# BloodAxe/segmentation-networks-benchmark

Measured on AMD Instinct MI355X. Metric: images/sec/GPU (fwd+bwd) ZF_UNET 224x224 bs=32; 1/2/4/8-GPU scaling, higher is better.
Workload: dtype bf16; 1 GPU; ZF_UNET 224x224 bf16 bs=32/GPU, bce_dice, SGD lr 1e-3, Dropout2d 0.2, train step torch_train.py:180-190 (configs[1]); global_batch=32, parallelism=dp1

## Files before the change

__graft_entry__.py:

```python
import os
import subprocess
import sys

ROOT = os.path.dirname(os.path.abspath(__file__))
PKG = os.path.join(ROOT, 'segmentation-networks-benchmark_amd')


def _paths():
    for p in (PKG, ROOT):
        if p not in sys.path:
            sys.path.insert(0, p)


def build():
    subprocess.check_call(['bash', os.path.join(PKG, 'csrc', 'build.sh')])
    _paths()
    import torch
    from segnb import _native as nv
    import ctypes
    lib = ctypes.CDLL(nv.LIB_PATH)
    for name in (list(nv.SIGNATURES) + list(nv.PLAIN) + list(nv.MC_SIGNATURES) + list(nv.MC_PLAIN) + list(nv.GCN_SIGNATURES)
                 + list(nv.GCN_PLAIN)):
        getattr(lib, name)
    import lib.models.zf_unet
    import lib.models.gcn
    import lib.losses
    import lib.metrics


def smoke():
    _paths()
    import torch
    from oracle import train_step_ref, zf_unet_ref
    from lib.models.zf_unet import ZF_UNET
    from lib.losses import BCEWithLogitsLossAndSmoothJaccard
    from segnb import _native as nv
    nv.load()
    dev = torch.device('cuda:0')
    B, S, F = 2, 64, 8
    x, y = train_step_ref.synthetic_batch(B, S, seed=21)
    sd = zf_unet_ref.default_init_state(filters=F, seed=5)
    ref_loss, ref_logits, ref_grads = train_step_ref.loss_and_grads(sd, x, y, 'bce_jaccard')
    torch.manual_seed(5)
    m = ZF_UNET(dropout_val=0.0, filters=F)
    m.set_compute_dtype('f32')
    m = m.to(dev).train()
    opt = torch.optim.SGD(m.parameters(), lr=1e-3)
    opt.zero_grad()
    out = m(x.to(dev))
    loss = BCEWithLogitsLossAndSmoothJaccard()(out, y.to(dev))
    (B * loss).backward()
    opt.step()
    torch.cuda.synchronize()
    dl = abs(loss.item() - ref_loss.item())
    assert dl < 1e-5, 'loss differs from the oracle by %g' % dl
    worst = 0.0
    for n, p in m.named_parameters():
        if n.endswith('.conv.bias'):
            assert float(p.grad.abs().max()) == 0.0
            continue
        r = ref_grads[n]
        worst = max(worst, float((p.grad.cpu() - r).abs().max() / (r.abs().max() + 1e-6)))
    assert worst < 2e-3, 'gradient differs from the oracle (rel %g)' % worst
    m2 = ZF_UNET(dropout_val=0.2, filters=F).to(dev).train()
    l2 = BCEWithLogitsLossAndSmoothJaccard()(m2(x.to(dev)), y.to(dev))
    (B * l2).backward()
    torch.cuda.synchronize()
    assert torch.isfinite(l2).item()
    print('smoke ok: |dloss| = %.2e, worst rel grad err = %.2e, bf16 loss = %.4f' % (dl, worst, l2.item()))


if __name__ == '__main__':
    build()
    if len(sys.argv) > 1 and sys.argv[1] == 'smoke':
        smoke()
```

segmentation-networks-benchmark_amd/csrc/common.h:

```cpp
#pragma once
#include <hip/hip_runtime.h>
#include <hip/hip_ext.h>
#include <stdint.h>
#include <stdio.h>
#include <string.h>

#include "../../include/segnb_hip.h"

typedef __attribute__((ext_vector_type(8))) __bf16 bf16x8_t;
typedef __attribute__((ext_vector_type(16))) float f32x16_t;

struct bf16_t {
    unsigned short bits;
};

void segnb_set_error(const char* fmt, ...);

#define SEGNB_CHECK_ARG(cond, msg)                                   \
    do {                                                             \
        if (!(cond)) {                                               \
            segnb_set_error("%s: bad argument: %s", __func__, msg);  \
            return SEGNB_E_BADARG;                                   \
        }                                                            \
    } while (0)
// ... 26 lines not shown
struct SegnbPlanScope {
    bool top;
    SegnbPlanScope();
    ~SegnbPlanScope();
};
template <class T>
inline T segnb_plan_keep(T v) {
    static_assert(!(std::is_pointer<T>::value && std::is_class<typename std::remove_pointer<T>::type>::value),
                  "segnb_plan_keep: add an overload that copies this struct into the plan");
    return v;
}
inline const segnb_conv_geom* segnb_plan_keep(const segnb_conv_geom* g) {
    return g ? (const segnb_conv_geom*)segnb_plan_dup(g, sizeof(*g)) : g;
}
inline const segnb_loss_spec* segnb_plan_keep(const segnb_loss_spec* g) {
    return g ? (const segnb_loss_spec*)segnb_plan_dup(g, sizeof(*g)) : g;
}
inline const segnb_bn_reduce_epilogue* segnb_plan_keep(const segnb_bn_reduce_epilogue* g) {
    return g ? (const segnb_bn_reduce_epilogue*)segnb_plan_dup(g, sizeof(*g)) : g;
}
inline const segnb_bn_apply_epilogue* segnb_plan_keep(const segnb_bn_apply_epilogue* g) {
    return g ? (const segnb_bn_apply_epilogue*)segnb_plan_dup(g, sizeof(*g)) : g;
}
inline const segnb_upcat_src* segnb_plan_keep(const segnb_upcat_src* g) {
    return g ? (const segnb_upcat_src*)segnb_plan_dup(g, sizeof(*g)) : g;
}
inline const segnb_operand_tf* segnb_plan_keep(const segnb_operand_tf* g) {
    return g ? (const segnb_operand_tf*)segnb_plan_dup(g, sizeof(*g)) : g;
}
inline const segnb_wgrad_target* segnb_plan_keep(const segnb_wgrad_target* g) {
    return g ? (const segnb_wgrad_target*)segnb_plan_dup(g, sizeof(*g)) : g;
}
inline const segnb_act_epilogue* segnb_plan_keep(const segnb_act_epilogue* g) {
    return g ? (const segnb_act_epilogue*)segnb_plan_dup(g, sizeof(*g)) : g;
}
template <class... P, class... A>
inline void segnb_plan_record_call(const char* name, int (*fn)(P...), A... args) {
    static_assert(sizeof...(P) == sizeof...(A), "argument count");
    std::tuple<P...> kept(segnb_plan_keep((P)args)...);
    segnb_plan_push([fn, kept]() { return std::apply(fn, kept); }, name);
}
extern int g_segnb_census_on;
void segnb_census(const char* name);
#define SEGNB_PLAN_RECORD(fn, ...)                                                           \
    SegnbPlanScope plan_scope__;                                                             \
    if (plan_scope__.top && g_segnb_census_on) segnb_census(#fn);                            \
    if (plan_scope__.top && segnb_plan_recording()) segnb_plan_record_call(#fn, fn, __VA_ARGS__)
void segnb_plan_refuse(const char* why);
#define SEGNB_PLAN_REFUSE(why)                                         \
    SegnbPlanScope plan_scope__;                                       \
    if (plan_scope__.top && g_segnb_census_on) segnb_census(__func__); \
    if (plan_scope__.top && segnb_plan_recording()) segnb_plan_refuse(why)

int segnb_num_cus();
int segnb_knob_fprop_dma();
int segnb_knob_fprop_dma_cfg();
int segnb_knob_fprop_dma_dbg();
int segnb_knob_fprop_nostats();
int segnb_knob_rw_store_waves();
int segnb_knob_bnreduce_fused();
int segnb_knob_fprop_deepk();
int segnb_knob_fprop_thin();
enum segnb_try_outcome {
    SEGNB_TRY_DECLINED = 0,
    SEGNB_TRY_LAUNCHED,
    SEGNB_TRY_DELIVERED,
};
inline int segnb_try_launched(segnb_try_outcome* did, int rc) {
    if (rc == 0) *did = SEGNB_TRY_LAUNCHED;
    return rc;
}
int segnb_fprop_thin_try(segnb_try_outcome* did, const segnb_conv_geom* g, const void* in, const void* wpacked, void* out,
                         hipStream_t stream, const segnb_bn_reduce_epilogue* bn);
int segnb_fprop_thin_ok(const segnb_conv_geom* g);
int segnb_knob_fprop_upd();
int segnb_knob_fprop_drop();
int segnb_knob_fprop_mask();
int segnb_fprop_dma_actmask_ok(const segnb_conv_geom* g);
int segnb_fprop_roll_actmask_ok(const segnb_conv_geom* g);
int segnb_knob_fprop_mf16();
int segnb_knob_fprop_rw();
int segnb_knob_fprop_ksplit();
float* segnb_head_scratch(size_t bytes, hipStream_t stream);
void segnb_head_bwd_finish(const float* part, int gx, int gy, int K, int C, int CT, float* dw, float* db, hipStream_t stream);
int segnb_knob_pack_blocks();
int segnb_knob_fprop_roll();
int segnb_knob_wg_cu_pct();
int segnb_knob_conv_cus();
int segnb_fprop_dma_read_stamps(unsigned long long* host_dst);
int segnb_fprop_s1_try(segnb_try_outcome* did, const segnb_conv_geom* g, const void* in, const void* wpacked, const float* bias, int bias_n,
                       void* out, double* stats, hipStream_t stream, const float* drop = nullptr, int ld_drop = 0, int stats_ld = 0);
int segnb_fprop_dma_try(segnb_try_outcome* did, const segnb_conv_geom* g, const void* in, unsigned in_bytes, const void* wpacked,
                        unsigned w_bytes, const float* bias, int bias_n, void* out, double* stats,
                        hipStream_t stream, const segnb_act_epilogue* ep = nullptr, const segnb_upcat_src* uc = nullptr,
                        const segnb_bn_reduce_epilogue* bn = nullptr);
int segnb_fprop_rw_try(segnb_try_outcome* did, const segnb_conv_geom* g, const void* in, unsigned in_bytes, const void* wpacked,
                       unsigned w_bytes, const float* bias, int bias_n, void* out, double* stats,
                       hipStream_t stream, const segnb_bn_reduce_epilogue* bn = nullptr,
                       const segnb_act_epilogue* ep = nullptr, const segnb_upcat_src* uc = nullptr,
                       const segnb_upcat_src* upsum = nullptr);
int segnb_fprop_roll_try(segnb_try_outcome* did, const segnb_conv_geom* g, const void* in, unsigned in_bytes, const void* wpacked,
                         unsigned w_bytes, const float* bias, int bias_n, void* out, double* stats, hipStream_t stream,
                         const segnb_bn_reduce_epilogue* bn = nullptr, const segnb_operand_tf* tf = nullptr,
                         const segnb_upcat_src* uc = nullptr);
int segnb_fprop_c8_try(segnb_try_outcome* did, const segnb_conv_geom* g, const void* in, const void* wpacked, const float* bias, int bias_n,
                       void* out, double* stats, hipStream_t stream, const segnb_act_epilogue* ep = nullptr);
struct segnb_wgrad_bnapply {
    const void* g;
    int ld_g;
    const void* y;
    int ld_y;
    const float* coef;
    const float* bcoef;
    int Cp;
    int act;
    float slope;
};
int segnb_wgrad_s1_try(segnb_try_outcome* did, const segnb_conv_geom* g, const void* in, const void* dout, float* dwp, int nslab,
                       hipStream_t stream, bool partial, const segnb_wgrad_bnapply* bna = nullptr,
                       const segnb_upcat_src* uc = nullptr, const segnb_wgrad_target* tgt = nullptr);
const segnb_wgrad_target* segnb_take_wgrad_target();
void segnb_wgrad_to_param(float* dwp, int Cop, int ntaps, int Cip, int nslab, const segnb_wgrad_target* tgt, bool rezero,
                          hipStream_t stream);
int segnb_wgrad_s1_slabs(const segnb_conv_geom* g);
void segnb_slab_reduce(float* dwp, long long total, int nslab, hipStream_t stream);
bool segnb_wgrad_roll_applies(const segnb_conv_geom* g);
int segnb_wgrad_roll_try(segnb_try_outcome* did, const segnb_conv_geom* g, const void* in, const void* dout, float* dwp, int nslab,
                         hipStream_t stream, bool partial, const segnb_operand_tf* tfx = nullptr, const segnb_operand_tf* tfd = nullptr);
int segnb_knob_wgrad_roll();
bool segnb_wgrad_c8roll_applies(const segnb_conv_geom* g);
int segnb_wgrad_c8roll_try(segnb_try_outcome* did, const segnb_conv_geom* g, const void* in, const void* dout, float* dwp, int nslab,
                           hipStream_t stream, bool partial, const segnb_wgrad_bnapply* bna = nullptr);
int segnb_knob_wgrad_c8roll();
int segnb_wgrad_sx_try(segnb_try_outcome* did, const segnb_conv_geom* g, const void* in, const void* dout, float* dwp, int nslab,
                       hipStream_t stream, bool partial);
int segnb_wgrad_sx_slabs(const segnb_conv_geom* g);
int segnb_fprop_upf_try(segnb_try_outcome* did, int N, int H, int W, int Ci, int ld_in, const void* in, unsigned in_bytes,
                        const void* wpacked, unsigned w_bytes, int Co, int CoW, void* out, int ld_out, double* stats,
                        hipStream_t stream, const float* bias = nullptr, int bias_n = 0, int no_prev = 0, int ep_act = -1,
                        float ep_slope = 0.f);
int segnb_fprop_sx_try(segnb_try_outcome* did, const segnb_conv_geom* g, const void* in, const void* wpacked, const float* bias,
                       int bias_n, void* out, double* stats, hipStream_t stream);

__device__ __forceinline__ float bf16_bits_to_f32(unsigned short b) {
    return __uint_as_float(((unsigned)b) << 16);
}
__device__ __forceinline__ unsigned short f32_to_bf16_bits(float f) {
    __bf16 h = (__bf16)f;
    return __builtin_bit_cast(unsigned short, h);
}

template <typename T>
struct Elem;
template <>
struct Elem<float> {
    static constexpr int EPC = 4;
    __device__ static __forceinline__ float to_f32(float v) { return v; }
    __device__ static __forceinline__ float from_f32(float v) { return v; }
    __device__ static __forceinline__ float round(float v) { return v; }
};
template <>
struct Elem<bf16_t> {
    static constexpr int EPC = 8;
    __device__ static __forceinline__ float to_f32(bf16_t v) { return bf16_bits_to_f32(v.bits); }
    __device__ static __forceinline__ bf16_t from_f32(float v) {
        bf16_t r;
// ... 53 lines not shown
```

segmentation-networks-benchmark_amd/csrc/head_loss.hip:

```cpp
#include "common.h"

#include <mutex>
#include <vector>

namespace {

constexpr int MAXK = 8;
constexpr int HEAD_MAXK = 32;

template <typename T, int KM = MAXK>
__global__ __launch_bounds__(256) void head_fwd_kernel(const T* __restrict__ a, int ld_a, long long npix,
                                                       long long hw, int C, const float* __restrict__ w,
                                                       const float* __restrict__ bias, int K,
                                                       float* __restrict__ logits) {
    extern __shared__ float sw[];
    const int C8 = (C + 7) & ~7;
    for (int i = threadIdx.x; i < K * C8; i += blockDim.x) {
        const int k = i / C8, c = i - k * C8;
        sw[i] = c < C ? w[k * C + c] : 0.f;
    }
    __syncthreads();
    for (long long pix = blockIdx.x * (long long)blockDim.x + threadIdx.x; pix < npix;
         pix += (long long)gridDim.x * blockDim.x) {
        float acc[KM];
#pragma unroll
        for (int k = 0; k < KM; ++k) acc[k] = 0.f;
        for (int c0 = 0; c0 < C8; c0 += 8) {
            float v[8];
            load8(a + pix * ld_a + c0, v);
#pragma unroll
            for (int k = 0; k < KM; ++k)
                if (k < K) {
#pragma unroll
                    for (int e = 0; e < 8; ++e) acc[k] = fmaf(v[e], sw[k * C8 + c0 + e], acc[k]);
                }
        }
        const long long n = pix / hw, r = pix - n * hw;
#pragma unroll
        for (int k = 0; k < KM; ++k)
            if (k < K) logits[(n * K + k) * hw + r] = acc[k] + (bias != nullptr ? bias[k] : 0.f);
    }
}

template <typename T, int KM>
__global__ __launch_bounds__(256) void head_fwd_wide_kernel(const T* __restrict__ a, int ld_a, long long npix, long long hw, int C,
                                                            const float* __restrict__ w, const float* __restrict__ bias, int K,
                                                            float* __restrict__ logits, int CT) {
    extern __shared__ float sww[];
    const int PY = 256 / CT;
    const int tx = threadIdx.x % CT, ty = threadIdx.x / CT;
    const int CPP = (C + 7) >> 3, C8 = CPP * 8;
    for (int i = threadIdx.x; i < K * C8; i += blockDim.x) {
        const int k = i / C8, c = i - k * C8;
        sww[i] = c < C ? w[k * C + c] : 0.f;
    }
    __syncthreads();
    for (long long pix = (long long)blockIdx.x * PY + ty; pix < npix; pix += (long long)gridDim.x * PY) {
        float acc[KM];
#pragma unroll
        for (int k = 0; k < KM; ++k) acc[k] = 0.f;
        for (int cc = tx; cc < CPP; cc += CT) {
            float v[8];
            load8(a + pix * ld_a + cc * 8, v);
#pragma unroll
            for (int k = 0; k < KM; ++k)
                if (k < K) {
                    const float4 w0 = *reinterpret_cast<const float4*>(sww + k * C8 + cc * 8);
                    const float4 w1 = *reinterpret_cast<const float4*>(sww + k * C8 + cc * 8 + 4);
                    acc[k] = fmaf(v[0], w0.x, acc[k]); acc[k] = fmaf(v[1], w0.y, acc[k]);
                    acc[k] = fmaf(v[2], w0.z, acc[k]); acc[k] = fmaf(v[3], w0.w, acc[k]);
                    acc[k] = fmaf(v[4], w1.x, acc[k]); acc[k] = fmaf(v[5], w1.y, acc[k]);
                    acc[k] = fmaf(v[6], w1.z, acc[k]); acc[k] = fmaf(v[7], w1.w, acc[k]);
                }
        }
#pragma unroll
        for (int k = 0; k < KM; ++k)
            for (int off = 1; off < CT; off <<= 1) acc[k] += __shfl_xor(acc[k], off);
        if (tx == 0) {
            const long long n = pix / hw, r = pix - n * hw;
#pragma unroll
            for (int k = 0; k < KM; ++k)
                if (k < K) logits[(n * K + k) * hw + r] = acc[k] + (bias != nullptr ? bias[k] : 0.f);
        }
// ... 324 lines not shown
                    }
                if (act >= 0) {
                    const float neg = act == SEGNB_ACT_RELU ? 0.f : (act == SEGNB_ACT_LEAKY ? slope : 1.f);
#pragma unroll
                    for (int e = 0; e < 8; ++e) {
                        const float gr = round_as(d[e], da);
                        d[e] = round_as(av[u][e] > 0.f ? gr : gr * neg, da);
                        sz[e] += d[e];
                    }
                }
                if (da != nullptr) store8(da + ioff[u] * ld_da + c0, d);
            }
        }
    }
    float* sg = sred;
    float* prow = part + (long long)(blockIdx.y * gridDim.x + blockIdx.x) * (KT * (CT * 8 + 1));
#pragma unroll
    for (int j = 0; j < KM; ++j)
        if (j < KT) {
            __syncthreads();
#pragma unroll
            for (int e = 0; e < 8; ++e) sg[(ty * CT + tx) * 8 + e] = gw[j][e];
            __syncthreads();
            if (threadIdx.x < CT * 8) {
                float sum = 0.f;
                for (int q = 0; q < PY; ++q) sum += sg[q * CT * 8 + threadIdx.x];
                prow[j * (CT * 8 + 1) + threadIdx.x] = sum;
            }
            __syncthreads();
            if (tx == 0) sg[ty] = gb[j];
            __syncthreads();
            if (threadIdx.x == 0 && j < K) {
                float sum = 0.f;
                for (int q = 0; q < PY; ++q) sum += sg[q];
                prow[(j * NT) * (CT * 8 + 1) + CT * 8] = sum;
            }
        }
    if (act >= 0 && sums != nullptr) {
        __syncthreads();
#pragma unroll
        for (int e = 0; e < 8; ++e) sg[(ty * CT + tx) * 8 + e] = sz[e];
        __syncthreads();
        if (threadIdx.x < CT * 8) {
            double sum = 0.0;
            for (int q = 0; q < PY; ++q) sum += (double)sg[q * CT * 8 + threadIdx.x];
            const int c = blockIdx.y * CT * 8 + threadIdx.x;
            if (c < Cp) atomicAdd(&sums[(long long)((blockIdx.x % SEGNB_STAT_REPLICAS) * 2) * Cp + c], sum);
        }
    }
}

__global__ __launch_bounds__(256) void head_bwd_finish_kernel(const float* __restrict__ part, int gx, int gy, int K, int C,
                                                              int CT, float* __restrict__ dw, float* __restrict__ db, int T) {
    __shared__ float sw4[4];
    const int o = blockIdx.x;
    const int t = threadIdx.x;
    const int row = K * (CT * 8 + 1);
    int k, by, idx;
    int c = 0;
    if (o < K * C) {
        k = o / C;
        c = o - k * C;
        by = c / (CT * 8);
        idx = c - by * (CT * 8);
    } else {
        k = (o - K * C) * T;
        by = 0;
        idx = CT * 8;
    }
    float sum = 0.f;
    for (int bx = t; bx < gx; bx += 256) sum += part[(long long)(by * gx + bx) * row + k * (CT * 8 + 1) + idx];
#pragma unroll
    for (int d = 32; d >= 1; d >>= 1) sum += __shfl_down(sum, d, 64);
    if ((t & 63) == 0) sw4[t >> 6] = sum;
    __syncthreads();
    if (t == 0) {
        const float tot = ((sw4[0] + sw4[1]) + sw4[2]) + sw4[3];
        if (o < K * C) {
            if (dw != nullptr) dw[((long long)(k / T) * C + c) * T + k % T] += tot;
        } else if (db != nullptr) {
            db[k / T] += tot;
        }
    }
}

struct PixTerms {
    float p;
    float e;
    float de;
    float f;
    float df;
};

__device__ __forceinline__ PixTerms pix_terms(float x, float t, float gamma = 2.f) {
    PixTerms o;
    const float ls = fminf(x, 0.f) - log1pf(expf(-fabsf(x)));
    const float p = expf(ls);
    o.p = p;
    o.e = -t * ls + log1pf(p);
    o.de = (1.f - p) * (p / (1.f + p) - t);
    const float pt = expf(-o.e);
    const float om = 1.f - pt;
    if (gamma == 2.f) {
        o.f = om * om * o.e;
        o.df = (2.f * om * pt * o.e + om * om) * o.de;
    } else if (om > 0.f) {
        const float pg1 = powf(om, gamma - 1.f), pg = pg1 * om;
        o.f = pg * o.e;
        o.df = (gamma * pg1 * pt * o.e + pg) * o.de;
    } else {
        o.f = gamma == 0.f ? o.e : 0.f;
        o.df = gamma == 0.f ? o.de : 0.f;
    }
    return o;
}

__device__ __forceinline__ void loss_finalize_math(const double* sums, const segnb_loss_spec& sp, float* __restrict__ out) {
    const double n = sums[6];
    const double I = sums[2], U = sums[3] + sums[4];
    const double bce = sp.bce_sum ? sums[0] : sums[0] / n;
    const double focal = sp.focal_mean ? sums[1] / n : sums[1];
    const double eps = (double)sp.eps, sm = (double)sp.smooth;
    const double Dj = U - I + eps, Ds = U - I + sm, Dd = U + eps;
    const double jac = 1.0 - I / Dj;
    const double sjac = 1.0 - (I + sm) / Ds;
    const double dice = 1.0 - 2.0 * I / Dd;
    const double loss = ((double)sp.w_bce * bce + (double)sp.w_focal * focal + (double)sp.w_jaccard * jac +
                         (double)sp.w_sjaccard * sjac + (double)sp.w_dice * dice) / (double)sp.norm;
    const double GI = (double)sp.w_jaccard * (-(U + eps) / (Dj * Dj)) + (double)sp.w_sjaccard * (-(U + 2.0 * sm) / (Ds * Ds)) +
                      (double)sp.w_dice * (-2.0 / Dd);
    const double GU = (double)sp.w_jaccard * (I / (Dj * Dj)) + (double)sp.w_sjaccard * ((I + sm) / (Ds * Ds)) +
                      (double)sp.w_dice * (2.0 * I / (Dd * Dd));
    out[0] = (float)loss;
    out[1] = (float)(I / (U - I + 1e-7));
    out[2] = (float)(sums[5] / n);
    out[3] = (float)GI;
    out[4] = (float)GU;
    out[5] = (float)bce;
    out[6] = (float)n;
    out[7] = 0.f;
}

constexpr int LOSS_REPL = 8;
template <bool FIN>
__global__ __launch_bounds__(256) void loss_reduce_kernel(const float* __restrict__ x,
                                                          const long long* __restrict__ tg, long long n,
                                                          double* __restrict__ sums, int vec, float gamma,
                                                          segnb_loss_spec sp, float* __restrict__ fin) {
    double s[6] = {0, 0, 0, 0, 0, 0};
    auto term = [&](float xv, long long tgv) {
        const float t = tgv != 0 ? 1.f : 0.f;
        const float tf = (float)tgv;
        const PixTerms q = pix_terms(xv, tf, gamma);
        s[0] += q.e;
        s[1] += q.f;
        s[2] += q.p * tf;
        s[3] += q.p;
        s[4] += tf;
        s[5] += ((q.p > 0.5f) == (t != 0.f)) ? 1.0 : 0.0;
    };
    const long long n4 = vec ? n / 4 : 0;
#pragma unroll 2
    for (long long j = blockIdx.x * (long long)blockDim.x + threadIdx.x; j < n4; j += (long long)gridDim.x * blockDim.x) {
        const float4 xv = reinterpret_cast<const float4*>(x)[j];
        const longlong2 t01 = reinterpret_cast<const longlong2*>(tg)[2 * j];
        const longlong2 t23 = reinterpret_cast<const longlong2*>(tg)[2 * j + 1];
        term(xv.x, t01.x);
        term(xv.y, t01.y);
        term(xv.z, t23.x);
        term(xv.w, t23.y);
    }
    for (long long i = 4 * n4 + blockIdx.x * (long long)blockDim.x + threadIdx.x; i < n;
         i += (long long)gridDim.x * blockDim.x)
        term(x[i], tg[i]);
    __shared__ double sh[4][6];
    const int lane = threadIdx.x & 63, wave = threadIdx.x >> 6;
#pragma unroll
    for (int k = 0; k < 6; ++k) {
        const double v = wave_sum(s[k]);
        if (lane == 0) sh[wave][k] = v;
    }
    __syncthreads();
    double* const dst = FIN ? sums + (blockIdx.x % LOSS_REPL) * 8 : sums;
    double ret = 0.0;
    if (threadIdx.x < 6) {
        const double v = sh[0][threadIdx.x] + sh[1][threadIdx.x] + sh[2][threadIdx.x] + sh[3][threadIdx.x];
        ret = atomicAdd(&dst[threadIdx.x], v);
    }
    if (threadIdx.x == 6 && blockIdx.x == 0) ret = atomicAdd(&dst[6], (double)n);
    if constexpr (FIN) {
        __shared__ int last;
        if (ret == -1.2345e300) fin[7] = 1.f;
        asm volatile("s_waitcnt vmcnt(0)" ::: "memory");
        __syncthreads();
        if (threadIdx.x == 0) {
            unsigned* ticket = reinterpret_cast<unsigned*>(sums + LOSS_REPL * 8);
            const unsigned tk = __hip_atomic_fetch_add(ticket, 1u, __ATOMIC_RELAXED, __HIP_MEMORY_SCOPE_AGENT);
            last = tk == gridDim.x - 1 ? 1 : 0;
            if (last) {
                __builtin_amdgcn_fence(__ATOMIC_ACQUIRE, "agent");
                asm volatile("s_waitcnt vmcnt(0)" ::: "memory");
            }
        }
        __syncthreads();
        if (last) {
            __shared__ double stot[LOSS_REPL * 8];
            if (threadIdx.x < LOSS_REPL * 8) {
                stot[threadIdx.x] = __hip_atomic_load(&sums[threadIdx.x], __ATOMIC_RELAXED, __HIP_MEMORY_SCOPE_AGENT);
                sums[threadIdx.x] = 0.0;
            }
            __syncthreads();
            if (threadIdx.x == 0) {
                double tot[7];
#pragma unroll
                for (int k = 0; k < 7; ++k) {
                    tot[k] = 0.0;
                    for (int rp = 0; rp < LOSS_REPL; ++rp) tot[k] += stot[rp * 8 + k];
                }
                loss_finalize_math(tot, sp, fin);
                *reinterpret_cast<unsigned*>(sums + LOSS_REPL * 8) = 0u;
            }
        }
    }
}

__global__ void loss_finalize_kernel(const double* __restrict__ sums, segnb_loss_spec sp, float* __restrict__ out) {
    if (threadIdx.x != 0 || blockIdx.x != 0) return;
    loss_finalize_math(sums, sp, out);
}

__global__ __launch_bounds__(256) void loss_bwd_kernel(const float* __restrict__ x, const long long* __restrict__ tg,
                                                       long long n, const float* __restrict__ fin, segnb_loss_spec sp,
                                                       const float* __restrict__ grad_out, float* __restrict__ dx,
                                                       int vec) {
    const float go = (grad_out != nullptr ? grad_out[0] : 1.f) / sp.norm;
    const float GI = fin[3], GU = fin[4];
    const float inv_n = 1.f / fin[6];
    const float wb = sp.bce_sum ? sp.w_bce : sp.w_bce * inv_n;
    const float wf = sp.focal_mean ? sp.w_focal * inv_n : sp.w_focal;
    auto grad = [&](float xv, long long tgv) {
        const float tf = (float)tgv;
        const PixTerms q = pix_terms(xv, tf, sp.focal_gamma);
        const float dp = q.p * (1.f - q.p);
        return go * (wb * q.de + wf * q.df + dp * (tf * GI + GU));
    };
    const long long n4 = vec ? n / 4 : 0;
    for (long long j = blockIdx.x * (long long)blockDim.x + threadIdx.x; j < n4; j += (long long)gridDim.x * blockDim.x) {
        const float4 xv = reinterpret_cast<const float4*>(x)[j];
        const longlong2 t01 = reinterpret_cast<const longlong2*>(tg)[2 * j];
        const longlong2 t23 = reinterpret_cast<const longlong2*>(tg)[2 * j + 1];
        float4 o;
        o.x = grad(xv.x, t01.x);
        o.y = grad(xv.y, t01.y);
        o.z = grad(xv.z, t23.x);
        o.w = grad(xv.w, t23.y);
        reinterpret_cast<float4*>(dx)[j] = o;
    }
    for (long long i = 4 * n4 + blockIdx.x * (long long)blockDim.x + threadIdx.x; i < n;
         i += (long long)gridDim.x * blockDim.x)
        dx[i] = grad(x[i], tg[i]);
}


__global__ __launch_bounds__(256) void loss_map_kernel(const float* __restrict__ x, const long long* __restrict__ tg,
                                                       long long n, int kind, float gamma, float* __restrict__ out) {
    for (long long i = blockIdx.x * (long long)blockDim.x + threadIdx.x; i < n; i += (long long)gridDim.x * blockDim.x) {
        const PixTerms q = pix_terms(x[i], (float)tg[i], gamma);
        out[i] = kind == 0 ? q.e : q.f;
    }
}

__global__ __launch_bounds__(256) void loss_map_bwd_kernel(const float* __restrict__ x, const long long* __restrict__ tg,
                                                           long long n, int kind, float gamma,
                                                           const float* __restrict__ gout, float* __restrict__ dx) {
    for (long long i = blockIdx.x * (long long)blockDim.x + threadIdx.x; i < n; i += (long long)gridDim.x * blockDim.x) {
        const PixTerms q = pix_terms(x[i], (float)tg[i], gamma);
        dx[i] = gout[i] * (kind == 0 ? q.de : q.df);
    }
}

__global__ __launch_bounds__(256) void absmax_kernel(const float* __restrict__ x, long long n, unsigned* __restrict__ out) {
    unsigned m = 0;
    const long long n4 = n / 4;
    for (long long j = blockIdx.x * (long long)blockDim.x + threadIdx.x; j < n4; j += (long long)gridDim.x * blockDim.x) {
        const uint4 v = reinterpret_cast<const uint4*>(x)[j];
        m = max(max(m, v.x & 0x7fffffffu), max(v.y & 0x7fffffffu, max(v.z & 0x7fffffffu, v.w & 0x7fffffffu)));
    }
    for (long long i = 4 * n4 + blockIdx.x * (long long)blockDim.x + threadIdx.x; i < n;
         i += (long long)gridDim.x * blockDim.x)
        m = max(m, __float_as_uint(x[i]) & 0x7fffffffu);
#pragma unroll
    for (int o = 32; o > 0; o >>= 1) m = max(m, (unsigned)__shfl_xor((int)m, o));
    if ((threadIdx.x & 63) == 0 && m != 0) atomicMax(out, m);
}

__global__ __launch_bounds__(256) void pr_hist_kernel(const float* __restrict__ x, const long long* __restrict__ tg,
                                                      long long n, const float* __restrict__ thr, int nthr,
                                                      unsigned long long* __restrict__ hist) {
    extern __shared__ unsigned sm[];
    unsigned* cnt = sm;
    float* th = reinterpret_cast<float*>(sm + 2 * (nthr + 1));
    for (int i = threadIdx.x; i < 2 * (nthr + 1); i += blockDim.x) cnt[i] = 0;
    for (int i = threadIdx.x; i < nthr; i += blockDim.x) th[i] = thr[i];
    __syncthreads();
    for (long long i = blockIdx.x * (long long)blockDim.x + threadIdx.x; i < n; i += (long long)gridDim.x * blockDim.x) {
        const float xv = x[i];
        const float p = expf(fminf(xv, 0.f) - log1pf(expf(-fabsf(xv))));
        int lo = 0, hi = nthr;
        while (lo < hi) {
            const int mid = (lo + hi) >> 1;
            if (th[mid] < p) lo = mid + 1; else hi = mid;
        }
        atomicAdd(&cnt[(tg[i] != 0 ? nthr + 1 : 0) + lo], 1u);
    }
    __syncthreads();
    for (int i = threadIdx.x; i < 2 * (nthr + 1); i += blockDim.x)
        if (cnt[i]) atomicAdd(&hist[i], (unsigned long long)cnt[i]);
}

}

extern "C" int segnb_head_fwd(int dtype, const void* a, int ld_a, int N, int H, int W, int C, const float* w,
                              const float* bias, int K, float* logits, segnb_stream_t stream) {
    SEGNB_PLAN_RECORD(segnb_head_fwd, dtype, a, ld_a, N, H, W, C, w, bias, K, logits, stream);
    SEGNB_CHECK_ARG(a && w && logits, "NULL tensor");
    SEGNB_CHECK_ARG(K >= 1 && K <= HEAD_MAXK, "head supports 1..32 classes");
    SEGNB_CHECK_ARG(N > 0 && H > 0 && W > 0 && C > 0 && ld_a % 8 == 0 && ld_a >= ((C + 7) & ~7), "bad shape");
    const long long npix = (long long)N * H * W;
    if (C > 64) {
        const int cpp = (C + 7) / 8;
        int ct = 1;
        while (ct < cpp && ct < 32) ct <<= 1;
        const int py = 256 / ct;
        long long gx = (npix + py - 1) / py;
        if (gx > 4096) gx = 4096;
        const size_t wsm = (size_t)K * cpp * 8 * sizeof(float);
        SEGNB_CHECK_ARG(wsm <= 48 * 1024, "head: K * C too large");
        if (dtype == SEGNB_BF16)
            (K == 1 ? head_fwd_wide_kernel<bf16_t, 1> : K <= MAXK ? head_fwd_wide_kernel<bf16_t, MAXK>
                                                    : K <= 16 ? head_fwd_wide_kernel<bf16_t, 16> : head_fwd_wide_kernel<bf16_t, HEAD_MAXK>)
                <<<dim3((unsigned)gx), dim3(256), wsm, (hipStream_t)stream>>>((const bf16_t*)a, ld_a, npix, (long long)H * W, C, w, bias, K,
                                                                             logits, ct);
        else if (dtype == SEGNB_F32)
            (K == 1 ? head_fwd_wide_kernel<float, 1> : K <= MAXK ? head_fwd_wide_kernel<float, MAXK>
                                                   : K <= 16 ? head_fwd_wide_kernel<float, 16> : head_fwd_wide_kernel<float, HEAD_MAXK>)
                <<<dim3((unsigned)gx), dim3(256), wsm, (hipStream_t)stream>>>((const float*)a, ld_a, npix, (long long)H * W, C, w, bias, K,
                                                                             logits, ct);
        else {
            segnb_set_error("segnb_head_fwd: unknown dtype %d", dtype);
            return SEGNB_E_BADARG;
        }
        SEGNB_LAUNCH_CHECK();
        return 0;
    }
    int grid = ceil_div(npix, 256);
    if (grid > 4096) grid = 4096;
    const int smem = K * ((C + 7) & ~7) * 4;
    SEGNB_CHECK_ARG(smem <= 60 * 1024, "head too wide");
    if (dtype == SEGNB_BF16 && K <= MAXK)
        hipLaunchKernelGGL(head_fwd_kernel<bf16_t>, dim3(grid), dim3(256), smem, (hipStream_t)stream,
                           (const bf16_t*)a, ld_a, npix, (long long)H * W, C, w, bias, K, logits);
    else if (dtype == SEGNB_F32 && K <= MAXK)
        hipLaunchKernelGGL(head_fwd_kernel<float>, dim3(grid), dim3(256), smem, (hipStream_t)stream, (const float*)a,
                           ld_a, npix, (long long)H * W, C, w, bias, K, logits);
    else if (dtype == SEGNB_BF16)
        hipLaunchKernelGGL((head_fwd_kernel<bf16_t, HEAD_MAXK>), dim3(grid), dim3(256), smem, (hipStream_t)stream,
                           (const bf16_t*)a, ld_a, npix, (long long)H * W, C, w, bias, K, logits);
    else if (dtype == SEGNB_F32)
        hipLaunchKernelGGL((head_fwd_kernel<float, HEAD_MAXK>), dim3(grid), dim3(256), smem, (hipStream_t)stream, (const float*)a,
                           ld_a, npix, (long long)H * W, C, w, bias, K, logits);
    else {
        segnb_set_error("segnb_head_fwd: unknown dtype %d", dtype);
        return SEGNB_E_BADARG;
    }
    SEGNB_LAUNCH_CHECK();
    return 0;
}

namespace {
float* head_scratch(size_t bytes, hipStream_t stream) {
    struct Ent {
        int dev;
        hipStream_t stream;
        float* buf;
        size_t cap;
    };
    static std::mutex mu;
    static std::vector<Ent> ents;
    int dev = 0;
    if (hipGetDevice(&dev) != hipSuccess) {
        segnb_set_error("segnb_head_bwd: hipGetDevice failed");
        return nullptr;
    }
    std::lock_guard<std::mutex> lock(mu);
    Ent* e = nullptr;
    for (auto& it : ents)
        if (it.dev == dev && it.stream == stream) e = &it;
    hipStreamCaptureStatus cap_st = hipStreamCaptureStatusNone;
    if ((e == nullptr || bytes > e->cap) && hipStreamIsCapturing(stream, &cap_st) == hipSuccess &&
        cap_st == hipStreamCaptureStatusActive) {
        for (auto& it : ents)
            if (it.dev == dev && it.cap >= bytes) return it.buf;
        segnb_set_error("segnb_head_bwd: no scratch buffer to capture with -- run one eager step before capturing a graph");
        return nullptr;
    }
    if (e == nullptr) {
        ents.push_back(Ent{dev, stream, nullptr, 0});
        e = &ents.back();
    }
    if (bytes > e->cap) {
        const size_t want = bytes < (1u << 20) ? (1u << 20) : bytes * 2;
        float* p = nullptr;
        if (hipMalloc(&p, want) != hipSuccess) {
            segnb_set_error("segnb_head_bwd: scratch allocation of %zu bytes failed", want);
            return nullptr;
        }
        e->buf = p;
        e->cap = want;
    }
    return e->buf;
}
}

float* segnb_head_scratch(size_t bytes, hipStream_t stream) { return head_scratch(bytes, stream); }
void segnb_head_bwd_finish(const float* part, int gx, int gy, int K, int C, int CT, float* dw, float* db, hipStream_t stream) {
    head_bwd_finish_kernel<<<dim3(K * C + K), dim3(256), 0, stream>>>(part, gx, gy, K, C, CT, dw, db, 1);
}

extern "C" int segnb_head_bwd(int dtype, const void* a, int ld_a, int N, int H, int W, int C, int Cp,
                              const float* w, int K, const float* dlogits, void* da, int ld_da, float* dw,
                              float* db, segnb_stream_t stream) {
    SEGNB_PLAN_RECORD(segnb_head_bwd, dtype, a, ld_a, N, H, W, C, Cp, w, K, dlogits, da, ld_da, dw, db, stream);
    SEGNB_CHECK_ARG(a && w && dlogits, "NULL tensor");
    SEGNB_CHECK_ARG(K >= 1 && K <= HEAD_MAXK, "head supports 1..32 classes");
    SEGNB_CHECK_ARG(N > 0 && H > 0 && W > 0 && C > 0 && Cp % 8 == 0 && Cp >= C, "bad shape");
    const long long npix = (long long)N * H * W;
    SEGNB_CHECK_ARG(npix < (1ll << 30), "pixel count exceeds the 32-bit index range");
    const int CPP = Cp / 8;
    int ct = 1;
    while (ct < CPP && ct < 32) ct <<= 1;
    const int gy = ceil_div(CPP, ct);
    const int py = 256 / ct;
    long long gx = (npix + py - 1) / py;
    if (gx > 2048 / gy) gx = 2048 / gy;
    if (gx < 1) gx = 1;
    const dim3 grid((unsigned)gx, (unsigned)gy);
    if (dtype != SEGNB_BF16 && dtype != SEGNB_F32) {
        segnb_set_error("segnb_head_bwd: unknown dtype %d", dtype);
        return SEGNB_E_BADARG;
    }
    float* part = head_scratch((size_t)gx * gy * K * (ct * 8 + 1) * sizeof(float), (hipStream_t)stream);
    if (part == nullptr) return SEGNB_E_BADARG;
    if (K > MAXK) {
        const dim3 gridz((unsigned)gx, (unsigned)gy, (unsigned)ceil_div(K, MAXK));
        const size_t wsm = (size_t)K * ct * 8 * sizeof(float);
        if (dtype == SEGNB_BF16)
            head_bwd_many_kernel<bf16_t><<<gridz, dim3(256), wsm, (hipStream_t)stream>>>(
                (const bf16_t*)a, ld_a, npix, (long long)H * W, C, Cp, w, K, dlogits, (bf16_t*)da, ld_da, part, ct);
        else
            head_bwd_many_kernel<float><<<gridz, dim3(256), wsm, (hipStream_t)stream>>>(
                (const float*)a, ld_a, npix, (long long)H * W, C, Cp, w, K, dlogits, (float*)da, ld_da, part, ct);
    } else if (dtype == SEGNB_BF16)
        (K == 1 ? head_bwd_kernel<bf16_t, 1> : head_bwd_kernel<bf16_t, MAXK>)<<<grid, dim3(256), 0, (hipStream_t)stream>>>(
            (const bf16_t*)a, ld_a, npix, (long long)H * W, C, Cp, w, K, dlogits, (bf16_t*)da, ld_da, part, ct);
    else
        (K == 1 ? head_bwd_kernel<float, 1> : head_bwd_kernel<float, MAXK>)<<<grid, dim3(256), 0, (hipStream_t)stream>>>(
            (const float*)a, ld_a, npix, (long long)H * W, C, Cp, w, K, dlogits, (float*)da, ld_da, part, ct);
    SEGNB_LAUNCH_CHECK();
    if (dw != nullptr || db != nullptr) {
        head_bwd_finish_kernel<<<dim3(K * C + K), dim3(256), 0, (hipStream_t)stream>>>(part, (int)gx, gy, K, C, ct, dw, db, 1);
        SEGNB_LAUNCH_CHECK();
    }
    return 0;
}


extern "C" int segnb_head_conv_ok(int C, int K, int kh, int kw) {
    return (K >= 1 && kh >= 1 && kw >= 1 && K * kh * kw <= MAXK && C >= 1 && C <= 64) ? 1 : 0;
}

extern "C" int segnb_head_conv_fwd(int dtype, const void* a, int ld_a, int N, int Hi, int Wi, int C, const float* w, int kh, int kw,
                                   int pad, const float* bias, int K, float* logits, segnb_stream_t stream) {
    SEGNB_PLAN_RECORD(segnb_head_conv_fwd, dtype, a, ld_a, N, Hi, Wi, C, w, kh, kw, pad, bias, K, logits, stream);
    SEGNB_CHECK_ARG(a && w && logits, "NULL tensor");
    SEGNB_CHECK_ARG(segnb_head_conv_ok(C, K, kh, kw), "classes x window positions <= 8 and C <= 64 (segnb_head_conv_ok)");
    SEGNB_CHECK_ARG(N > 0 && Hi > 0 && Wi > 0 && pad >= 0 && ld_a % 8 == 0 && ld_a >= ((C + 7) & ~7), "bad shape");
    const int Ho = Hi + 2 * pad - kh + 1, Wo = Wi + 2 * pad - kw + 1;
    SEGNB_CHECK_ARG(Ho > 0 && Wo > 0, "empty output");
    const long long npix = (long long)N * Ho * Wo;
    SEGNB_CHECK_ARG(npix < (1ll << 30) && (long long)N * Hi * Wi < (1ll << 30), "pixel count exceeds the 32-bit index range");
    const int cpp = (C + 7) / 8;
    int ct = 1;
    while (ct < cpp) ct <<= 1;
    const int py = 256 / ct;
    long long gx = (npix + py - 1) / py;
    if (gx > 16384) gx = 16384;
    const int grid = (int)gx;
    const int smem = K * kh * kw * cpp * 8 * 4;
    const int nt = kh * kw;
#define SEGNB_HEAD_CONV_FWD(TT, NTM_)                                                                                         \
    hipLaunchKernelGGL((head_conv_fwd_kernel<TT, NTM_>), dim3(grid), dim3(256), smem, (hipStream_t)stream, (const TT*)a, ld_a, N, Hi, \
                       Wi, C, w, kh, kw, pad, bias, K, Ho, Wo, logits, ct)
    if (dtype == SEGNB_BF16) {
        if (nt == 1) SEGNB_HEAD_CONV_FWD(bf16_t, 1);
        else if (nt <= 4) SEGNB_HEAD_CONV_FWD(bf16_t, 4);
        else SEGNB_HEAD_CONV_FWD(bf16_t, MAXK);
    } else if (dtype == SEGNB_F32) {
// ... 169 lines not shown
```

segmentation-networks-benchmark_amd/csrc/norm_act.hip:

```cpp
#include "common.h"

namespace {

constexpr int NTHR = 256;
constexpr int REPL = SEGNB_STAT_REPLICAS;

struct EwShape {
    int N, H, W, Cp;
    int CPP;
    int CT;
    int PY;
};

static EwShape make_shape(int N, int H, int W, int Cp) {
    EwShape s;
    s.N = N; s.H = H; s.W = W; s.Cp = Cp;
    s.CPP = Cp / 8;
    int ct = 1;
    while (ct < s.CPP && ct < 32) ct <<= 1;
    s.CT = ct;
    s.PY = NTHR / ct;
    return s;
}

static dim3 make_grid(const EwShape& s, long long items, int max_blocks = 2048) {
    const int gy = ceil_div(s.CPP, s.CT);
    long long gx = (items + s.PY - 1) / s.PY;
    long long cap = max_blocks / gy;
    if (cap < 1) cap = 1;
    if (gx > cap) gx = cap;
    const long long want = (items + 4ll * s.PY - 1) / (4ll * s.PY);
    if (gx > want) gx = want;
    if (gx < 1) gx = 1;
    return dim3((unsigned)gx, (unsigned)gy);
}

__device__ __forceinline__ float act_neg_scale(int act, float slope) {
    return act == SEGNB_ACT_RELU ? 0.f : (act == SEGNB_ACT_LEAKY ? slope : 1.f);
}
__device__ __forceinline__ float act_fwd(float z, int act, float slope) {
    return (z > 0.f ? z : z * act_neg_scale(act, slope)) + 0.f;
}
__device__ __forceinline__ float act_grad(float z, int act, float slope) {
    return z > 0.f ? 1.f : act_neg_scale(act, slope);
}

struct BnFwdParams {
    const double* stats;
    double count;
    const float* gamma;
    const float* beta;
    float eps, momentum;
    float* running_mean;
    float* running_var;
    long long* nbt;
    int C, training;
    float* coef;
    double* zero_buf;
    int keep_stats;
    int stats_ld;
};

__device__ __forceinline__ void bn_fwd_coef(const BnFwdParams& p, int Cp, int c, bool update, float& scale,
                                            float& shift, float& mean, float& invstd) {
    scale = shift = mean = invstd = 0.f;
    if (c >= p.C) return;
    double mu, var;
    if (p.training) {
        double v1[REPL], v2[REPL];
        const int SL = p.stats_ld > 0 ? p.stats_ld : Cp;
#pragma unroll
        for (int rp = 0; rp < REPL; ++rp) {
            v1[rp] = p.stats[(rp * 2) * SL + c];
            v2[rp] = p.stats[(rp * 2 + 1) * SL + c];
        }
        double s1 = 0.0, s2 = 0.0;
#pragma unroll
        for (int rp = 0; rp < REPL; ++rp) {
            s1 += v1[rp];
            s2 += v2[rp];
        }
        mu = s1 / p.count;
        var = s2 / p.count - mu * mu;
// ... 638 lines not shown
                    if (pooled) unpack_raw(rgp[i], gp);
#pragma unroll
                    for (int r = 0; r < 2; ++r)
#pragma unroll
                        for (int e = 0; e < 8; ++e)
                            a[r][e] = dm[e] * act_fwd((yv[r][e] - mu[e]) * sc[e] + sh[e], act, slope);
                    if constexpr (sizeof(T) == 2) {
                        const unsigned prio_t = 3u - (unsigned)dx, prio_b = 1u - (unsigned)dx;
#pragma unroll
                        for (int e = 0; e < 8; e += 2) {
                            const unsigned pt = pack2bf(a[0][e], a[0][e + 1]), pb = pack2bf(a[1][e], a[1][e + 1]);
#pragma unroll
                            for (int h = 0; h < 2; ++h) {
                                const unsigned bt = h ? pt >> 16 : pt & 0xffffu, bb = h ? pb >> 16 : pb & 0xffffu;
                                const unsigned kt = (bf16_order_key(bt, nonneg) << 2) | prio_t;
                                const unsigned kb = (bf16_order_key(bb, nonneg) << 2) | prio_b;
                                const unsigned kpt = __shfl_xor(kt, s.CT), kpb = __shfl_xor(kb, s.CT);
                                const unsigned mo = max(kpt, kpb);
                                if (pooled && kt > max(mo, kb)) g[0][e + h] += gp[e + h];
                                if (pooled && kb > max(mo, kt)) g[1][e + h] += gp[e + h];
                            }
                        }
                    } else {
#pragma unroll
                        for (int e = 0; e < 8; ++e) {
                            const float ptop = __shfl_xor(a[0][e], s.CT), pbot = __shfl_xor(a[1][e], s.CT);
                            const float a0 = dx ? ptop : a[0][e], a1 = dx ? a[0][e] : ptop;
                            const float a2 = dx ? pbot : a[1][e], a3 = dx ? a[1][e] : pbot;
                            int am = 0;
                            float m = a0;
                            if (a1 > m) { m = a1; am = 1; }
                            if (a2 > m) { m = a2; am = 2; }
                            if (a3 > m) { m = a3; am = 3; }
                            if (pooled && am == dx) g[0][e] += gp[e];
                            if (pooled && am == 2 + dx) g[1][e] += gp[e];
                        }
                    }
                }
#pragma unroll
                for (int r = 0; r < NR; ++r) {
                    if constexpr (HAS_U) {
                        if (okr[i][r]) {
#pragma unroll
                            for (int q = 0; q < 4; ++q) {
                                float t[8];
                                unpack_raw(ru[i][r][q], t);
#pragma unroll
                                for (int e = 0; e < 8; ++e) g[r][e] += t[e];
                            }
                        }
                    }
                    if (!(live && okr[i][r])) continue;
                    float rv[8];
#pragma unroll
                    for (int e = 0; e < 8; ++e) rv[e] = 0.f;
                    long long pix;
                    if constexpr (HAS_P) {
                        pix = ((long long)pn[i] * s.H + 2 * ph[i] + r) * s.W + pw[i];
                    } else {
                        pix = it0 + i * stride;
                        if constexpr (RES) unpack_raw(rres[i], rv);
                    }
                    bwd_pixel_math<T, APPLY>(yv[r], sc, sh, mu, dm, act, slope, g[r], rv,
                                             dz != nullptr ? dz + pix * ld_dz + c0 : (T*)nullptr, s1, s2, ap);
                }
            }
            it0 += U * stride;
            if (it0 < total) issue(it0);
        }
    }
    if (!APPLY && sums != nullptr) {
        if (coef != nullptr) {
#pragma unroll
            for (int e = 0; e < 8; ++e) s2[e] *= coef[3 * s.Cp + c0 + e];
        } else {
#pragma unroll
            for (int e = 0; e < 8; ++e) s2[e] = 0.f;
        }
        double* rep = sums + (long long)(blockIdx.x % REPL) * 2 * s.Cp;
        block_channel_sum2(s1, s2, s, tx, blockIdx.y * s.CT, rep, rep + s.Cp, sred);
    }
}

template <typename T, int KM>
__global__ __launch_bounds__(NTHR) void head_bn_bwd_kernel(const T* __restrict__ y, int ld_y, EwShape s,
                                                           const float* __restrict__ coef, int act, float slope,
                                                           const float* __restrict__ dropmul, const float* __restrict__ w, int C,
                                                           int K, const float* __restrict__ dl, T* __restrict__ dz, int ld_dz,
                                                           double* __restrict__ sums, float* __restrict__ part) {
    __shared__ float sred[SRED_FLOATS];
    constexpr int U = 2;
    const int tx = threadIdx.x % s.CT, ty = threadIdx.x / s.CT;
    const int cc = blockIdx.y * s.CT + tx;
    const bool active = cc < s.CPP;
    const int c0 = active ? cc * 8 : 0;
    const int stride = gridDim.x * s.PY;
    const int npix = s.N * s.H * s.W, hw = s.H * s.W;
    const FastDiv d_hw(hw);
    float wv[KM][8], gw[KM][8], gb[KM];
#pragma unroll
    for (int k = 0; k < KM; ++k) {
        gb[k] = 0.f;
#pragma unroll
        for (int e = 0; e < 8; ++e) {
            wv[k][e] = (k < K && c0 + e < C) ? w[k * C + c0 + e] : 0.f;
            gw[k][e] = 0.f;
        }
    }
    float sc[8], sh[8], mu[8], s1[8], s2[8];
    load8(coef + c0, sc);
    load8(coef + s.Cp + c0, sh);
    load8(coef + 2 * s.Cp + c0, mu);
#pragma unroll
    for (int e = 0; e < 8; ++e) s1[e] = s2[e] = 0.f;
    if (active) {
        for (int it0 = blockIdx.x * s.PY + ty; it0 < npix; it0 += U * stride) {
            Raw8<T> ry[U];
            Raw8<float> rdm[U];
            float g[U][KM];
#pragma unroll
            for (int u = 0; u < U; ++u) {
                const int pix = it0 + u * stride;
                const int pc = pix < npix ? pix : it0;
                load_raw(y + (long long)pc * ld_y + c0, ry[u]);
                const int n = (dropmul != nullptr || KM > 1) ? d_hw.div(pc) : 0;
                if (dropmul != nullptr) load_raw(dropmul + n * s.Cp + c0, rdm[u]);
                if (KM == 1) {
                    g[u][0] = dl[pc];
                } else {
                    const int r = pc - n * hw;
#pragma unroll
                    for (int k = 0; k < KM; ++k) g[u][k] = k < K ? dl[((long long)n * K + k) * hw + r] : 0.f;
                }
            }
#pragma unroll
            for (int u = 0; u < U; ++u) {
                const int pix = it0 + u * stride;
                if (pix >= npix) break;
                float yv[8], dm[8], a[8], d[8], yc[8], z[8];
                unpack_raw(ry[u], yv);
#pragma unroll
                for (int e = 0; e < 8; ++e) dm[e] = 1.f;
                if (dropmul != nullptr) unpack_raw(rdm[u], dm);
#pragma unroll
                for (int e = 0; e < 8; ++e) {
                    yc[e] = yv[e] - mu[e];
                    z[e] = yc[e] * sc[e] + sh[e];
                    a[e] = dm[e] * act_fwd(z[e], act, slope);
                    d[e] = 0.f;
                }
                round_store8((T*)nullptr, a);
#pragma unroll
                for (int k = 0; k < KM; ++k)
                    if (k < K) {
                        const float gk = g[u][k];
                        gb[k] += gk;
#pragma unroll
                        for (int e = 0; e < 8; ++e) {
                            d[e] = fmaf(gk, wv[k][e], d[e]);
                            gw[k][e] = fmaf(gk, a[e], gw[k][e]);
                        }
                    }
                round_store8((T*)nullptr, d);
#pragma unroll
                for (int e = 0; e < 8; ++e) d[e] = d[e] * dm[e] * act_grad(z[e] + 0.f, act, slope);
                round_store8(dz != nullptr ? dz + (long long)pix * ld_dz + c0 : (T*)nullptr, d);
#pragma unroll
                for (int e = 0; e < 8; ++e) {
                    s1[e] += d[e];
                    s2[e] += d[e] * yc[e];
                }
            }
        }
    }
#pragma unroll
    for (int e = 0; e < 8; ++e) s2[e] *= coef[3 * s.Cp + c0 + e];
    double* rep = sums + (long long)(blockIdx.x % REPL) * 2 * s.Cp;
    block_channel_sum2(s1, s2, s, tx, blockIdx.y * s.CT, rep, rep + s.Cp, sred);
    const int CT = s.CT, PY = s.PY;
    float* sg = sred;
    float* prow = part + (long long)(blockIdx.y * gridDim.x + blockIdx.x) * (K * (CT * 8 + 1));
#pragma unroll
    for (int k = 0; k < KM; ++k)
        if (k < K) {
            __syncthreads();
#pragma unroll
            for (int e = 0; e < 8; ++e) sg[(ty * CT + tx) * 8 + e] = gw[k][e];
            __syncthreads();
            if ((int)threadIdx.x < CT * 8) {
                float sum = 0.f;
                for (int j = 0; j < PY; ++j) sum += sg[j * CT * 8 + threadIdx.x];
                prow[k * (CT * 8 + 1) + threadIdx.x] = sum;
            }
            __syncthreads();
            if (tx == 0) sg[ty] = gb[k];
            __syncthreads();
            if (threadIdx.x == 0) {
                float sum = 0.f;
                for (int j = 0; j < PY; ++j) sum += sg[j];
                prow[k * (CT * 8 + 1) + CT * 8] = sum;
            }
        }
}


template <typename T, int KM>
__global__ __launch_bounds__(NTHR) void head_bn_apply_kernel(const T* __restrict__ y, int ld_y, EwShape s,
                                                             const float* __restrict__ coef, int act, float slope,
                                                             const float* __restrict__ dropmul, const float* __restrict__ w, int C,
                                                             int K, const float* __restrict__ dl, T* __restrict__ dy, int ld_dy,
                                                             const BnBwdParams bp) {
    __shared__ float sred[SRED_FLOATS];
    constexpr int U = 2;
    const int tx = threadIdx.x % s.CT, ty = threadIdx.x / s.CT;
    const int cc = blockIdx.y * s.CT + tx;
    const bool active = cc < s.CPP;
    const int c0 = active ? cc * 8 : 0;
    const int stride = gridDim.x * s.PY;
    const int npix = s.N * s.H * s.W, hw = s.H * s.W;
    const FastDiv d_hw(hw);
    Raw8<T> ry[U];
    Raw8<float> rdm[U];
    float g[U][KM];
    auto issue = [&](int it0) {
#pragma unroll
        for (int u = 0; u < U; ++u) {
            const int pix = it0 + u * stride;
            const int pc = pix < npix ? pix : it0;
            load_raw(y + (long long)pc * ld_y + c0, ry[u]);
            const int n = (dropmul != nullptr || KM > 1) ? d_hw.div(pc) : 0;
            if (dropmul != nullptr) load_raw(dropmul + n * s.Cp + c0, rdm[u]);
            if (KM == 1) {
                g[u][0] = dl[pc];
            } else {
                const int r = pc - n * hw;
#pragma unroll
                for (int k = 0; k < KM; ++k) g[u][k] = k < K ? dl[((long long)n * K + k) * hw + r] : 0.f;
            }
        }
    };
    int it0 = blockIdx.x * s.PY + ty;
    if (active && it0 < npix) issue(it0);
    float ap[4][8];
    apply_src_coefs(bp, coef, s, tx, c0, sred, ap);
    float wv[KM][8];
#pragma unroll
    for (int k = 0; k < KM; ++k)
#pragma unroll
        for (int e = 0; e < 8; ++e) wv[k][e] = (k < K && c0 + e < C) ? w[k * C + c0 + e] : 0.f;
    float sc[8], sh[8], mu[8];
    load8(coef + c0, sc);
    load8(coef + s.Cp + c0, sh);
    load8(coef + 2 * s.Cp + c0, mu);
    if (!active) return;
    while (it0 < npix) {
#pragma unroll
        for (int u = 0; u < U; ++u) {
            const int pix = it0 + u * stride;
            if (pix >= npix) break;
            float yv[8], dm[8], d[8], yc[8], z[8];
            unpack_raw(ry[u], yv);
#pragma unroll
            for (int e = 0; e < 8; ++e) dm[e] = 1.f;
            if (dropmul != nullptr) unpack_raw(rdm[u], dm);
#pragma unroll
            for (int e = 0; e < 8; ++e) {
                yc[e] = yv[e] - mu[e];
                z[e] = yc[e] * sc[e] + sh[e];
                d[e] = 0.f;
            }
#pragma unroll
            for (int k = 0; k < KM; ++k)
                if (k < K) {
                    const float gk = g[u][k];
#pragma unroll
                    for (int e = 0; e < 8; ++e) d[e] = fmaf(gk, wv[k][e], d[e]);
                }
            round_store8((T*)nullptr, d);
#pragma unroll
            for (int e = 0; e < 8; ++e) d[e] = d[e] * dm[e] * act_grad(z[e] + 0.f, act, slope);
            round_store8((T*)nullptr, d);
#pragma unroll
            for (int e = 0; e < 8; ++e) {
                const float yh = yc[e] * ap[3][e];
                d[e] = ap[0][e] * (d[e] - ap[1][e] - yh * ap[2][e]);
            }
            round_store8(dy + (long long)pix * ld_dy + c0, d);
        }
        it0 += U * stride;
        if (it0 < npix) issue(it0);
    }
}


__global__ void bn_bwd_finalize_kernel(const BnBwdParams p, const float* __restrict__ coef, int Cp) {
    const int c = blockIdx.x * blockDim.x + threadIdx.x;
    if (c >= Cp) return;
    float a, c1, c2;
    bn_bwd_coef(p, coef, Cp, c, true, a, c1, c2);
    if (c < p.C) {
        double* sm = const_cast<double*>(p.sums);
#pragma unroll
        for (int rp = 0; rp < REPL; ++rp) {
            sm[(rp * 2) * Cp + c] = 0.0;
            sm[(rp * 2 + 1) * Cp + c] = 0.0;
        }
    }
    p.bcoef[c] = a;
    p.bcoef[Cp + c] = c1;
    p.bcoef[2 * Cp + c] = c2;
    if (p.zero_buf != nullptr) {
#pragma unroll
        for (int rp = 0; rp < REPL; ++rp) {
            p.zero_buf[(rp * 2) * Cp + c] = 0.0;
            p.zero_buf[(rp * 2 + 1) * Cp + c] = 0.0;
        }
    }
}

__device__ __forceinline__ float bn_dz_elem(float d, float yv, float mu, float sc, float sh, int act, float slope) {
    return d * 1.f * act_grad((yv - mu) * sc + sh + 0.f, act, slope);
}
__device__ __forceinline__ float bn_apply_elem(float yv, float d, float mu, float is, float a, float c1, float c2) {
    const float yh = (yv - mu) * is;
    return a * (d - c1 - yh * c2);
}

template <typename T, bool ACC = false>
__global__ __launch_bounds__(NTHR) void bn_bwd_apply_kernel(const T* __restrict__ y, int ld_y, EwShape s,
                                                            const float* __restrict__ coef,
                                                            const float* __restrict__ bcoef,
                                                            const T* __restrict__ dz, int ld_dz, T* __restrict__ dy,
                                                            int ld_dy, float* __restrict__ dbias, int C,
                                                            const BnBwdParams bp, const T* __restrict__ g, int ld_g,
                                                            int act, float slope) {
    __shared__ float sred[32 * 8];
    __shared__ float sb3[3][32 * 8];
    for (int i = threadIdx.x; i < 32 * 8; i += NTHR) sred[i] = 0.f;
// ... 518 lines not shown
    SEGNB_PLAN_RECORD(segnb_bn_act_bwd_reduce, dtype, y, ld_y, N, H, W, Cp, coef, act, slope, dropmul, g_direct, ld_gd, g_pool, ld_gp, g_up, ld_gu, dz, ld_dz, sums, res, ld_res, stream);
    if (int rc = check_ew(N, H, W, Cp)) return rc;
    SEGNB_CHECK_ARG(y != nullptr, "NULL tensor");
    SEGNB_CHECK_ARG(g_direct || g_pool || g_up, "no gradient source");
    SEGNB_CHECK_ARG(dz != nullptr || sums != nullptr, "a pass without dz needs the sums (the apply pass recomputes dz: "
                    "segnb_bn_bwd_apply_direct / segnb_bn_bwd_apply_fused_src)");
    SEGNB_CHECK_ARG(!(res && g_pool), "residual input and pooled gradient cannot be combined");
    const EwShape s = make_shape(N, H, W, Cp);
    const bool hd = g_direct != nullptr, hp = g_pool != nullptr, hu = g_up != nullptr;
    const long long items = hp ? (long long)N * ((H + 1) / 2) * (2 * ((W + 1) / 2)) : (long long)N * H * W;
    const dim3 grid = make_grid(s, items);
    const int variant = (hd ? 1 : 0) | (hp ? 2 : 0) | (hu ? 4 : 0);
#define SEGNB_RED(TT, D, P, U, R)                                                                                   \
    SEGNB_LAUNCH_FORKABLE((bn_act_bwd_reduce_kernel<TT, D, P, U, false, R>), grid, dim3(NTHR), 0, (hipStream_t)stream, \
                       (const TT*)y, ld_y, s, coef, act, slope, dropmul, (const TT*)g_direct, ld_gd,              \
                       (const TT*)g_pool, ld_gp, (const TT*)g_up, ld_gu, (TT*)dz, ld_dz, sums, (const TT*)res, ld_res, BnBwdParams{})
#define SEGNB_RED_R(TT, D, U)                                                                                       \
    if (res != nullptr) SEGNB_RED(TT, D, false, U, true); else SEGNB_RED(TT, D, false, U, false)
#define SEGNB_RED_ALL(TT)                                                       \
    switch (variant) {                                                          \
        case 1: SEGNB_RED_R(TT, true, false); break;                            \
        case 2: SEGNB_RED(TT, false, true, false, false); break;                \
        case 3: SEGNB_RED(TT, true, true, false, false); break;                 \
        case 4: SEGNB_RED_R(TT, false, true); break;                            \
        case 5: SEGNB_RED_R(TT, true, true); break;                             \
        case 6: SEGNB_RED(TT, false, true, true, false); break;                 \
        default: SEGNB_RED(TT, true, true, true, false); break;                 \
    }
    if (dtype == SEGNB_BF16) {
        SEGNB_RED_ALL(bf16_t)
    } else if (dtype == SEGNB_F32) {
        SEGNB_RED_ALL(float)
    } else {
        segnb_set_error("segnb_bn_act_bwd_reduce: unknown dtype %d", dtype);
        return SEGNB_E_BADARG;
    }
#undef SEGNB_RED_ALL
#undef SEGNB_RED_R
#undef SEGNB_RED
    SEGNB_LAUNCH_CHECK();
    return 0;
}

extern "C" int segnb_bn_act_bwd_reduce_add(int dtype, const void* y, int ld_y, int N, int H, int W, int Cp, const float* coef, int act,
                                           float slope, const float* dropmul, const void* g_direct, int ld_gd, const void* g_add,
                                           int ld_ga, void* dz, int ld_dz, double* sums, const void* res, int ld_res,
                                           segnb_stream_t stream) {
    SEGNB_PLAN_RECORD(segnb_bn_act_bwd_reduce_add, dtype, y, ld_y, N, H, W, Cp, coef, act, slope, dropmul, g_direct, ld_gd, g_add, ld_ga, dz, ld_dz, sums, res, ld_res, stream);
    if (int rc = check_ew(N, H, W, Cp)) return rc;
    SEGNB_CHECK_ARG(y != nullptr && g_direct != nullptr && g_add != nullptr, "NULL tensor");
    SEGNB_CHECK_ARG(dz != nullptr || sums != nullptr, "a pass without dz needs the sums");
    const EwShape s = make_shape(N, H, W, Cp);
    const dim3 grid = make_grid(s, (long long)N * H * W);
#define SEGNB_RED_A(TT, R)                                                                                                     \
    SEGNB_LAUNCH_FORKABLE((bn_act_bwd_reduce_kernel<TT, true, false, false, false, R, true>), grid, dim3(NTHR), 0, (hipStream_t)stream, \
                          (const TT*)y, ld_y, s, coef, act, slope, dropmul, (const TT*)g_direct, ld_gd, (const TT*)nullptr, 0,    \
                          (const TT*)g_add, ld_ga, (TT*)dz, ld_dz, sums, (const TT*)res, ld_res, BnBwdParams{})
    if (dtype == SEGNB_BF16) {
        if (res != nullptr) SEGNB_RED_A(bf16_t, true); else SEGNB_RED_A(bf16_t, false);
    } else if (dtype == SEGNB_F32) {
        if (res != nullptr) SEGNB_RED_A(float, true); else SEGNB_RED_A(float, false);
    } else {
        segnb_set_error("segnb_bn_act_bwd_reduce_add: unknown dtype %d", dtype);
        return SEGNB_E_BADARG;
    }
#undef SEGNB_RED_A
    SEGNB_LAUNCH_CHECK();
    return 0;
}

extern "C" int segnb_head_bn_bwd(int dtype, const void* y, int ld_y, int N, int H, int W, int C, int Cp, const float* coef,
                                 int act, float slope, const float* dropmul, const float* head_w, int K, const float* dlogits,
                                 void* dz, int ld_dz, double* sums, float* dw, float* db, segnb_stream_t stream) {
    SEGNB_PLAN_RECORD(segnb_head_bn_bwd, dtype, y, ld_y, N, H, W, C, Cp, coef, act, slope, dropmul, head_w, K, dlogits, dz, ld_dz, sums, dw, db, stream);
    if (int rc = check_ew(N, H, W, Cp)) return rc;
    SEGNB_CHECK_ARG(y && coef && head_w && dlogits && sums && C > 0 && Cp >= C, "NULL tensor");
    SEGNB_CHECK_ARG(segnb_head_fused_ok(K, Cp), "1..4 classes, Cp / 8 a power of two <= 32 (segnb_head_fused_ok)");
    const EwShape s = make_shape(N, H, W, Cp);
    const dim3 grid = make_grid(s, (long long)N * H * W);
    float* part = segnb_head_scratch((size_t)grid.x * grid.y * K * (s.CT * 8 + 1) * sizeof(float), (hipStream_t)stream);
    if (part == nullptr) return SEGNB_E_BADARG;
#define SEGNB_HBB(TT, KMM)                                                                                          \
    hipLaunchKernelGGL((head_bn_bwd_kernel<TT, KMM>), grid, dim3(NTHR), 0, (hipStream_t)stream, (const TT*)y, ld_y, s, coef, \
                       act, slope, dropmul, head_w, C, K, dlogits, (TT*)dz, ld_dz, sums, part)
    if (dtype == SEGNB_BF16) {
        if (K == 1) SEGNB_HBB(bf16_t, 1); else SEGNB_HBB(bf16_t, 4);
    } else if (dtype == SEGNB_F32) {
        if (K == 1) SEGNB_HBB(float, 1); else SEGNB_HBB(float, 4);
    } else {
        segnb_set_error("segnb_head_bn_bwd: unknown dtype %d", dtype);
        return SEGNB_E_BADARG;
    }
#undef SEGNB_HBB
    SEGNB_LAUNCH_CHECK();
    if (dw != nullptr || db != nullptr) {
        segnb_head_bwd_finish(part, (int)grid.x, (int)grid.y, K, C, s.CT, dw, db, (hipStream_t)stream);
        SEGNB_LAUNCH_CHECK();
    }
    return 0;
}

extern "C" int segnb_head_bn_bwd_apply(int dtype, const void* y, int ld_y, int N, int H, int W, int C, int Cp, const float* coef,
                                       const double* sums, const float* gamma, float* bcoef, float* dgamma, float* dbeta,
                                       int accumulate, double* fwd_stats_to_clear, int act, float slope, const float* dropmul,
                                       const float* head_w, int K, const float* dlogits, void* dy, int ld_dy,
                                       segnb_stream_t stream) {
    SEGNB_PLAN_RECORD(segnb_head_bn_bwd_apply, dtype, y, ld_y, N, H, W, C, Cp, coef, sums, gamma, bcoef, dgamma, dbeta, accumulate,
                      fwd_stats_to_clear, act, slope, dropmul, head_w, K, dlogits, dy, ld_dy, stream);
    if (int rc = check_ew(N, H, W, Cp)) return rc;
    SEGNB_CHECK_ARG(y && coef && sums && bcoef && head_w && dlogits && dy && C > 0 && Cp >= C, "NULL tensor");
    SEGNB_CHECK_ARG(segnb_head_fused_ok(K, Cp), "1..4 classes, Cp / 8 a power of two <= 32 (segnb_head_fused_ok)");
    SEGNB_CHECK_ARG(ld_y % 8 == 0 && ld_dy % 8 == 0 && ld_y >= Cp && ld_dy >= Cp, "bad strides");
    const EwShape s = make_shape(N, H, W, Cp);
    const dim3 grid = make_grid(s, (long long)N * H * W);
    const BnBwdParams bp = {sums, (double)N * H * W, gamma, dgamma, dbeta, C, accumulate, bcoef, fwd_stats_to_clear};
#define SEGNB_HBA(TT, KMM)                                                                                                    \
    SEGNB_LAUNCH_FORKABLE((head_bn_apply_kernel<TT, KMM>), grid, dim3(NTHR), 0, (hipStream_t)stream, (const TT*)y, ld_y, s, coef, \
                          act, slope, dropmul, head_w, C, K, dlogits, (TT*)dy, ld_dy, bp)
    if (dtype == SEGNB_BF16) {
        if (K == 1) SEGNB_HBA(bf16_t, 1); else SEGNB_HBA(bf16_t, 4);
    } else if (dtype == SEGNB_F32) {
        if (K == 1) SEGNB_HBA(float, 1); else SEGNB_HBA(float, 4);
    } else {
        segnb_set_error("segnb_head_bn_bwd_apply: unknown dtype %d", dtype);
        return SEGNB_E_BADARG;
    }
#undef SEGNB_HBA
    SEGNB_LAUNCH_CHECK();
    return 0;
}

struct BiasGradJob {
    double* sums;
    float* gb;
    int C, Cp;
};
__global__ __launch_bounds__(256) void bias_grad_multi_kernel(const BiasGradJob* __restrict__ jobs) {
    const BiasGradJob j = jobs[blockIdx.x];
    for (int c = threadIdx.x; c < j.Cp; c += blockDim.x) {
        double v[REPL];
#pragma unroll
        for (int rp = 0; rp < REPL; ++rp) v[rp] = j.sums[(rp * 2) * j.Cp + c];
        double t = 0.0;
#pragma unroll
        for (int rp = 0; rp < REPL; ++rp) t += v[rp];
        if (c < j.C && j.gb != nullptr) j.gb[c] += (float)t;
#pragma unroll
        for (int rp = 0; rp < REPL; ++rp) {
            j.sums[(rp * 2) * j.Cp + c] = 0.0;
            j.sums[(rp * 2 + 1) * j.Cp + c] = 0.0;
        }
    }
}

extern "C" int segnb_bias_grad_job_bytes(void) { return (int)sizeof(BiasGradJob); }

extern "C" int segnb_bias_grad_multi(const void* jobs, int njobs, segnb_stream_t stream) {
    SEGNB_PLAN_RECORD(segnb_bias_grad_multi, jobs, njobs, stream);
    SEGNB_CHECK_ARG(jobs != nullptr && njobs > 0, "bad job table");
    hipLaunchKernelGGL(bias_grad_multi_kernel, dim3(njobs), dim3(256), 0, (hipStream_t)stream, (const BiasGradJob*)jobs);
    SEGNB_LAUNCH_CHECK();
    return 0;
}

extern "C" int segnb_bn_bwd_finalize(double* sums, int C, int Cp, double count, const float* gamma,
                                     const float* coef, float* bcoef, float* dgamma, float* dbeta,
                                     int accumulate, segnb_stream_t stream) {
    SEGNB_PLAN_RECORD(segnb_bn_bwd_finalize, sums, C, Cp, count, gamma, coef, bcoef, dgamma, dbeta, accumulate, stream);
    SEGNB_CHECK_ARG(sums && coef && bcoef && C > 0 && Cp >= C && Cp % 8 == 0, "bad arguments");
    BnBwdParams bp = {sums, count, gamma, dgamma, dbeta, C, accumulate, bcoef, nullptr};
    hipLaunchKernelGGL(bn_bwd_finalize_kernel, dim3(ceil_div(Cp, 64)), dim3(64), 0, (hipStream_t)stream, bp, coef, Cp);
    SEGNB_LAUNCH_CHECK();
    return 0;
}

extern "C" int segnb_bn_bwd_finalize_clear(double* sums, int C, int Cp, double count, const float* gamma,
                                           const float* coef, float* bcoef, float* dgamma, float* dbeta,
                                           int accumulate, double* fwd_stats_to_clear, segnb_stream_t stream) {
    SEGNB_PLAN_RECORD(segnb_bn_bwd_finalize_clear, sums, C, Cp, count, gamma, coef, bcoef, dgamma, dbeta, accumulate, fwd_stats_to_clear, stream);
    SEGNB_CHECK_ARG(sums && coef && bcoef && C > 0 && Cp >= C && Cp % 8 == 0, "bad arguments");
    BnBwdParams bp = {sums, count, gamma, dgamma, dbeta, C, accumulate, bcoef, fwd_stats_to_clear};
    hipLaunchKernelGGL(bn_bwd_finalize_kernel, dim3(ceil_div(Cp, 64)), dim3(64), 0, (hipStream_t)stream, bp, coef, Cp);
    SEGNB_LAUNCH_CHECK();
    return 0;
}

static int launch_bn_bwd_apply(int dtype, const void* y, int ld_y, int N, int H, int W, int Cp, const float* coef,
                               const float* bcoef, const void* dz, int ld_dz, void* dy, int ld_dy, float* dbias, int C,
                               const BnBwdParams& bp, const char* who, segnb_stream_t stream, const void* g = nullptr,
                               int ld_g = 0, int act = 0, float slope = 0.f, bool acc = false) {
    if (int rc = check_ew(N, H, W, Cp)) return rc;
    SEGNB_CHECK_ARG(y && coef && (bcoef || bp.bcoef) && (dz || g) && dy, "NULL tensor");
    const EwShape s = make_shape(N, H, W, Cp);
    const dim3 grid = make_grid(s, (long long)N * H * W, 1536);
    if (acc && dtype == SEGNB_BF16)
        SEGNB_LAUNCH_FORKABLE((bn_bwd_apply_kernel<bf16_t, true>), grid, dim3(NTHR), 0, (hipStream_t)stream, (const bf16_t*)y,
                           ld_y, s, coef, bcoef, (const bf16_t*)dz, ld_dz, (bf16_t*)dy, ld_dy, dbias, C, bp,
                           (const bf16_t*)g, ld_g, act, slope);
    else if (acc && dtype == SEGNB_F32)
        SEGNB_LAUNCH_FORKABLE((bn_bwd_apply_kernel<float, true>), grid, dim3(NTHR), 0, (hipStream_t)stream, (const float*)y,
                           ld_y, s, coef, bcoef, (const float*)dz, ld_dz, (float*)dy, ld_dy, dbias, C, bp,
                           (const float*)g, ld_g, act, slope);
    else if (dtype == SEGNB_BF16)
        SEGNB_LAUNCH_FORKABLE(bn_bwd_apply_kernel<bf16_t>, grid, dim3(NTHR), 0, (hipStream_t)stream, (const bf16_t*)y,
                           ld_y, s, coef, bcoef, (const bf16_t*)dz, ld_dz, (bf16_t*)dy, ld_dy, dbias, C, bp,
                           (const bf16_t*)g, ld_g, act, slope);
    else if (dtype == SEGNB_F32)
        SEGNB_LAUNCH_FORKABLE(bn_bwd_apply_kernel<float>, grid, dim3(NTHR), 0, (hipStream_t)stream, (const float*)y,
                           ld_y, s, coef, bcoef, (const float*)dz, ld_dz, (float*)dy, ld_dy, dbias, C, bp,
                           (const float*)g, ld_g, act, slope);
// ... 471 lines not shown
```

segmentation-networks-benchmark_amd/lib/models/zf_unet.py:

```python
import contextlib
import os

import torch
from torch import nn

from segnb import _native as nv
from segnb import convplan as cp
from segnb.launchlist import Recorder
from segnb.engine import ConvOp, FlatParams, InputNorm, PackTable, Runtime, Stage, UpCatConvOp, View, pack_input

ENCODER = ('conv_224', 'conv_112', 'conv_56', 'conv_28', 'conv_14', 'conv_7')
DECODER = ('up_conv_14', 'up_conv_28', 'up_conv_56', 'up_conv_112', 'up_conv_224')


class _ConvUnit(nn.Module):

    def __init__(self, cin, cout, bn):
        super(_ConvUnit, self).__init__()
        self.conv = nn.Conv2d(cin, cout, 3, padding=1)
        self.bn = nn.BatchNorm2d(cout) if bn else None
        self.activation = nn.ReLU(inplace=True)

    def forward(self, x):
        raise RuntimeError('sub-blocks are parameter holders; run the whole ZF_UNET (fused HIP plan)')
# ... 393 lines not shown
        ckey = None if u8 else self._cplan_key('fwd', N, H, W, train, need_grad, drop)
        first = None
        if u8 and self.stages[ENCODER[0]][0].conv.u8_direct_ok(N, H, W, self.wp[0]):
            first = (x, self.module.input_norm)
        else:
            pack_input(rt, x, b['x'], self.module.input_norm)
        if ckey is not None:
            for n in ENCODER + DECODER:
                for st in self.stages[n]:
                    if st.bn is not None and train and st.bnl.stats_left:
                        st.bnl.stats.zero_()
                        st.bnl.stats_left = False
            plan = self._cplans.get(ckey)
            self._guard_active = self._guard_f.begin()
            if plan is not None and plan[0] is not None:
                self._guard_mode = (ckey, 'replay')
                self._plan_replay(plan)
                self._last = (N, H, W) if need_grad else None
                self._last_train = bool(train)
                self.generation += 1
                return self._head(b, N, H, W, hf)
            if plan is not None:
                ckey = None
        with self._recording(ckey):
            wp = self.wp
            cur = b['x']
            for i, name in enumerate(ENCODER):
                s1, s2 = self.stages[name]
                defer = self._defer(s1, s2, cur, b['a1_%d' % i], train, need_grad)
                y1 = s1.forward(cur, train, None, out=b['a1_%d' % i], need_grad=need_grad, u8=first if i == 0 else None,
                                defer_act=defer)
                x2, tf2 = (y1, s1.tf_out()) if defer else (b['a1_%d' % i], None)
                if i < 5:
                    skip = b['cat_%d' % i].slice(wp[i + 1], wp[i])
                    s2.forward(x2, train, drop[name], out=skip, pool_out=b['p_%d' % (i + 1)], need_grad=need_grad, x_tf=tf2)
                    cur = b['p_%d' % (i + 1)]
                else:
                    s2.forward(b['a1_%d' % i], train, drop[name], need_grad=need_grad,
                               up_out=b['cat_4'].slice(0, wp[5]) if self._upsampled(4, N, H, W) else None, out=b.get('u_4'))
            for name, lvl in zip(DECODER, (4, 3, 2, 1, 0)):
                s1, s2 = self.stages[name]
                if self.subpixel:
                    s1.conv.bind_up(b.get('u_%d' % lvl), b.get('du_%d' % lvl))
                defer = self._defer(s1, s2, b['cat_%d' % lvl], b['b1_%d' % lvl], train, need_grad)
                y1 = s1.forward(b['cat_%d' % lvl], train, None, out=b['b1_%d' % lvl], need_grad=need_grad, defer_act=defer)
                x2, tf2 = (y1, s1.tf_out()) if defer else (b['b1_%d' % lvl], None)
                if lvl > 0:
                    s2.forward(x2, train, drop[name], need_grad=need_grad,
                               up_out=(b['cat_%d' % (lvl - 1)].slice(0, wp[lvl]) if self._upsampled(lvl - 1, N, H, W) else None),
                               out=b.get('u_%d' % (lvl - 1)), x_tf=tf2)
                elif hf:
                    s2.forward(x2, train, drop[name], need_grad=need_grad, x_tf=tf2, defer_act='head')
                else:
                    s2.forward(x2, train, drop[name], out=b['f0'], need_grad=need_grad, x_tf=tf2)
        self._last = (N, H, W) if need_grad else None
        self.generation += 1
        self._last_train = bool(train)
        return self._head(b, N, H, W, hf)

    HEAD_FUSION = os.environ.get('SEGNB_HEAD_FUSION', '1') != '0'

    def _head_fusable(self, train, need_grad):
        s2 = self.stages[DECODER[-1]][1]
        return bool(self.HEAD_FUSION and train and need_grad and s2.bn is not None and s2.fuse_finalize
                    and nv.query('segnb_head_fused_ok', self.K, self.wp[0]))

    def _defer(self, s1, s2, x1, a1, train, need_grad):
        if self.rt.code != nv.BF16 or not s1.defer_act_ok(x1, train, need_grad) or not isinstance(s2.conv, ConvOp):
            return False
        y = s1.buffers(x1.N, a1.H, a1.W)['y']
        y2 = s2.buffers(x1.N, a1.H, a1.W)['y']
        return s2.conv.fprop_tf_ok(y, y2) and s2.conv.wgrad_tf_ok(y, y2)

    def _head(self, b, N, H, W, fused=False):
        from segnb import seglosses
        rt = self.rt
        head = self.module.conv_final
        logits = torch.empty((N, self.K, H, W), dtype=torch.float32, device=rt.device)
        if fused:
            self.stages[DECODER[-1]][1].head_forward(head.weight.detach(), head.bias.detach(), self.K, logits)
        else:
            nv.call('segnb_head_fwd', rt.code, b['f0'].ptr, b['f0'].ld, N, H, W, self.widths[0],
                    nv.ptr(head.weight.detach()), nv.ptr(head.bias.detach()), self.K, nv.ptr(logits), rt.stream)
        seglosses.register_grad_buffer(logits, b['dlogits_in'])
        return logits

    def backward(self, dlogits):
        self._guard_mode, self._guard_active = (None, None), False
        out = self._backward(dlogits)
        self._guard_b.end(self._guard_active, *self._guard_mode)
        return out

    def _backward(self, dlogits):
        rt, flat, wp = self.rt, self.flat, self.wp
        if self._last is None:
            raise RuntimeError('backward without a grad-enabled forward')
        if not self._last_train and self.module._cfg['bn']:
            raise RuntimeError('backward through an eval-mode forward is not supported: BatchNorm gradients are '
                               'implemented for training mode (call model.train(), or run the forward under no_grad)')
        N, H, W = self._last
        b = self.buffers(N, H, W)
        accumulate_in_place = flat.begin_backward()
        with rt.weight_grads(store=not accumulate_in_place):
            return self._backward_lists(dlogits, b, N, H, W, accumulate_in_place)

    def _backward_lists(self, dlogits, b, N, H, W, accumulate_in_place):
        rt, flat, wp = self.rt, self.flat, self.wp
        drop_now = {n: self.stages[n][1]._saved[2] if self.stages[n][1]._saved is not None else None for n in ENCODER + DECODER}
        ckey = self._cplan_key('bwd', N, H, W, True, True, drop_now)
        if ckey is not None:
            ckey = ckey + (bool(getattr(self, '_last_head_fused', False)), bool(accumulate_in_place))
        if ckey is not None:
            din = b['dlogits_in']
            if dlogits.data_ptr() != din.data_ptr():
                din.copy_(dlogits)
            dlogits = din
            plan = self._cplans.get(ckey)
            self._guard_active = self._guard_b.begin()
            if plan is not None and plan[0] is not None:
                self._guard_mode = (ckey, 'replay')
                self._plan_replay(plan, H, W)
                rt._side_busy = False
                self._after_backward()
                flat.publish_grads(accumulate_in_place)
                return [None] * len(flat._off)
            if plan is not None:
                ckey = None
        with self._recording(ckey):
            if self._dg_pack_on_side and rt.side_stream() is not None:
                nv.call('segnb_stream_join', rt.stream, rt.side_stream().cuda_stream)
            head = self.module.conv_final
            hf = bool(getattr(self, '_last_head_fused', False))
            if hf:
                self.stages[DECODER[-1]][1].head_backward(head.weight.detach(), self.K, dlogits, flat.grad_of(head.weight),
                                                          flat.grad_of(head.bias))
            else:
                nv.call('segnb_head_bwd', rt.code, b['f0'].ptr, b['f0'].ld, N, H, W, self.widths[0], wp[0],
                        nv.ptr(head.weight.detach()), self.K, nv.ptr(dlogits), b['df0'].ptr, b['df0'].ld,
                        nv.ptr(flat.grad_of(head.weight)), nv.ptr(flat.grad_of(head.bias)), rt.stream)
            for name, lvl in zip(reversed(DECODER), (0, 1, 2, 3, 4)):
                s1, s2 = self.stages[name]
                if lvl == 0 and hf:
                    red = s2.backward(flat, dx=b['db1_0'], fuse_reduce_of=s1, dz_ready=True)
                elif lvl == 0:
                    red = s2.backward(flat, g_direct=b['df0'], dx=b['db1_0'], fuse_reduce_of=s1)
                elif self._seg(lvl - 1, N, H, W):
                    red = s2.backward(flat, g_direct=b['du_%d' % (lvl - 1)], dx=b['db1_%d' % lvl], fuse_reduce_of=s1)
                else:
                    red = s2.backward(flat, g_up=b['dcat_%d' % (lvl - 1)].slice(0, wp[lvl]), dx=b['db1_%d' % lvl],
                                      fuse_reduce_of=s1)
                if self.subpixel:
                    s1.conv.bind_up(b.get('u_%d' % lvl), b.get('du_%d' % lvl))
                s1.backward(flat, g_direct=b['db1_%d' % lvl], dx=b['dcat_%d' % lvl], reduced=red)
            self._unpack_group(H, W, 0)
            for i in (5, 4, 3, 2, 1, 0):
                if i == 3:
                    self._unpack_group(H, W, 1)
                s1, s2 = self.stages[ENCODER[i]]
                if i == 5 and self._seg(4, N, H, W):
                    red = s2.backward(flat, g_direct=b['du_4'], dx=b['da1_5'], fuse_reduce_of=s1)
                elif i == 5:
                    red = s2.backward(flat, g_up=b['dcat_4'].slice(0, wp[5]), dx=b['da1_5'], fuse_reduce_of=s1)
                else:
                    red = s2.backward(flat, g_direct=b['dcat_%d' % i].slice(wp[i + 1], wp[i]), g_pool=b['dp_%d' % (i + 1)],
                                      dx=b['da1_%d' % i], fuse_reduce_of=s1)
                s1.backward(flat, g_direct=b['da1_%d' % i], dx=(b['dp_%d' % i] if i > 0 else None), reduced=red)
            rt.join_side()
            self._tables(H, W)[2][2].run()
        self._after_backward()
        flat.publish_grads(accumulate_in_place)
        return [None] * len(flat._off)

    def _after_backward(self):
        hook = getattr(self.module, '_grad_sync_hook', None)
        if hook is not None:
            hook(self.flat)
```

segmentation-networks-benchmark_amd/segnb/_native.py:

```python
import ctypes
import os

MAX_TAPS = 64
F32, BF16 = 0, 1
ACT_NONE, ACT_RELU, ACT_LEAKY = 0, 1, 2

_HERE = os.path.dirname(os.path.abspath(__file__))
LIB_PATH = os.environ.get('SEGNB_LIB') or os.path.join(os.path.dirname(_HERE), 'csrc', 'libsegnb_hip.so')

c_int, c_float, c_double, c_void_p, c_ll = (ctypes.c_int, ctypes.c_float, ctypes.c_double, ctypes.c_void_p,
                                            ctypes.c_longlong)


class ConvGeom(ctypes.Structure):
    _fields_ = [('N', c_int), ('Hi', c_int), ('Wi', c_int), ('Ci', c_int),
                ('Ho', c_int), ('Wo', c_int), ('Co', c_int),
                ('ld_in', c_int), ('ld_out', c_int),
                ('QH', c_int), ('QW', c_int),
                ('in_step', c_int), ('out_step', c_int),
                ('oh0', c_int), ('ow0', c_int),
                ('ntaps', c_int),
                ('dh', c_int * MAX_TAPS), ('dw', c_int * MAX_TAPS)]


# ... 101 lines not shown
    'segnb_bn_bwd_apply_fused_direct_acc': [c_int, _P, c_int, c_int, c_int, c_int, c_int, c_int, _P, _P, _P, _P, _P, _P, c_int,
                                        _P, c_int, c_float, _P, c_int, _P, c_int, _P],
    'segnb_bn_bwd_apply_fused_src': [c_int, _P, c_int, c_int, c_int, c_int, c_int, c_int, _P, _P, _P, _P, _P, _P, c_int, _P,
                                     c_int, c_float, _P, _P, c_int, _P, c_int, _P, c_int, _P, c_int, _P],
    'segnb_abn_scale': [_P, c_float, _P, c_int, _P],
    'segnb_abn_dscale': [_P, _P, _P, c_int, _P],
    'segnb_tiles_gather': [_P, c_int, c_int, c_int, c_int, c_int, _P, c_int, c_int, c_int, _P, _P],
    'segnb_tiles_gather_u8': [_P, c_int, c_int, c_int, c_int, c_int, _P, c_int, c_int, c_int, c_float,
                              ctypes.POINTER(c_float), ctypes.POINTER(c_float), _P, _P],
    'segnb_tiles_merge': [_P, c_int, c_int, _P, c_int, c_int, c_int, c_int, _P, c_int, c_int, c_int, c_int, _P, _P],
    'segnb_add': [c_int, _P, c_int, _P, c_int, _P, c_int, c_int, c_int, c_int, c_int, _P],
    'segnb_bn_stats': [c_int, _P, c_int, c_int, c_int, c_int, c_int, _P, _P],
    'segnb_upsample_bilinear2x_fwd': [c_int, _P, c_int, c_int, c_int, c_int, c_int, _P, c_int, _P],
    'segnb_upsample_bilinear2x_bwd': [c_int, _P, c_int, c_int, c_int, c_int, c_int, _P, c_int, _P],
    'segnb_maxpool_fwd': [c_int, _P, c_int, c_int, c_int, c_int, c_int, c_int, c_int, c_int, _P, c_int, _P, _P],
    'segnb_maxpool_bwd': [c_int, _P, c_int, _P, c_int, c_int, c_int, c_int, c_int, c_int, c_int, c_int, _P, c_int, _P, _P],
    'segnb_maxpool_bwd_add': [c_int, _P, c_int, _P, c_int, _P, c_int, c_int, c_int, c_int, c_int, c_int, c_int, c_int, _P, c_int, _P, _P],
    'segnb_nhwc_to_nchw_f32': [c_int, _P, c_int, c_int, c_int, c_int, c_int, _P, _P],
    'segnb_bn_bwd_finalize': [_P, c_int, c_int, c_double, _P, _P, _P, _P, _P, c_int, _P],
    'segnb_bn_bwd_finalize_clear': [_P, c_int, c_int, c_double, _P, _P, _P, _P, _P, c_int, _P, _P],
    'segnb_bn_bwd_apply_direct': [c_int, _P, c_int, c_int, c_int, c_int, c_int, _P, _P, c_int, c_float, _P, c_int, _P, c_int,
                                  _P, c_int, _P],
    'segnb_bn_bwd_apply': [c_int, _P, c_int, c_int, c_int, c_int, c_int, _P, _P, _P, c_int, _P, c_int, _P, c_int,
                           _P],
    'segnb_head_fwd': [c_int, _P, c_int, c_int, c_int, c_int, c_int, _P, _P, c_int, _P, _P],
    'segnb_head_bwd': [c_int, _P, c_int, c_int, c_int, c_int, c_int, c_int, _P, c_int, _P, _P, c_int, _P, _P, _P],
    'segnb_head_conv_fwd': [c_int, _P, c_int, c_int, c_int, c_int, c_int, _P, c_int, c_int, c_int, _P, c_int, _P, _P],
    'segnb_head_conv_bwd': [c_int, _P, c_int, c_int, c_int, c_int, c_int, c_int, _P, c_int, c_int, c_int, c_int, _P, c_int, c_float,
                            _P, c_int, _P, _P, _P, _P],
    'segnb_seg_loss_reduce': [_P, _P, c_ll, c_float, _P, _P],
    'segnb_seg_loss_reduce_finalize': [_P, _P, c_ll, ctypes.POINTER(LossSpec), _P, _P, _P],
    'segnb_seg_loss_map': [_P, _P, c_ll, c_int, c_float, _P, _P],
    'segnb_seg_loss_map_bwd': [_P, _P, c_ll, c_int, c_float, _P, _P, _P],
    'segnb_absmax_f32': [_P, c_ll, _P, _P],
    'segnb_pr_histogram': [_P, _P, c_ll, _P, c_int, _P, _P],
    'segnb_seg_loss_finalize': [_P, ctypes.POINTER(LossSpec), _P, _P],
    'segnb_seg_loss_bwd': [_P, _P, c_ll, _P, _P, ctypes.POINTER(LossSpec), _P, _P, _P],
    'segnb_tune': [ctypes.c_char_p, c_int],
    'segnb_wg_cu_share': [c_int],
    'segnb_plan_begin': [],
    'segnb_plan_end': [ctypes.POINTER(c_void_p), ctypes.POINTER(c_int)],
    'segnb_plan_run': [_P],
    'segnb_plan_destroy': [_P],
    'segnb_stream_fork': [_P, _P],
    'segnb_stream_fork_arm': [_P],
    'segnb_stream_fork_commit': [_P, _P],
    'segnb_event_record': [_P, _P],
    'segnb_stream_join': [_P, _P],
    'segnb_debug_stamps': [_P],
    'segnb_debug_census': [ctypes.c_char_p, c_int],
    'segnb_sgd_step': [_P, _P, c_ll, c_float, _P],
    'segnb_rmsprop_step': [_P, _P, _P, c_ll, c_float, c_float, c_float, _P],
    'segnb_adam_step': [_P, _P, _P, _P, c_ll, c_float, c_float, c_float, c_float, c_int, _P],
}
PLAIN = {'segnb_version': (c_int, []), 'segnb_pack_pair_job_bytes': (c_int, []), 'segnb_pack_pair_job_blocks': (c_int, [c_int, c_int, c_int, c_int]), 'segnb_pack_elem_job_blocks': (c_int, [c_int, c_int, c_int]), 'segnb_bias_grad_job_bytes': (c_int, []), 'segnb_head_fused_ok': (c_int, [c_int, c_int]), 'segnb_head_conv_ok': (c_int, [c_int, c_int, c_int, c_int]), 'segnb_conv_fprop_tf_ok': (c_int, [ctypes.POINTER(ConvGeom), c_int, c_int]), 'segnb_conv_wgrad_tf_ok': (c_int, [ctypes.POINTER(ConvGeom), c_int]), 'segnb_conv_fprop_bnreduce_ok': (c_int, [ctypes.POINTER(ConvGeom), c_int]), 'segnb_conv_fprop_actmask_ok': (c_int, [ctypes.POINTER(ConvGeom), c_int]), 'segnb_conv_fprop_drop_ok': (c_int, [ctypes.POINTER(ConvGeom), c_int]), 'segnb_conv_fprop_bnapply_ok': (c_int, [ctypes.POINTER(ConvGeom), c_int]), 'segnb_conv_fprop_u8_ok': (c_int, [ctypes.POINTER(ConvGeom), c_int]), 'segnb_conv_fprop_upd_ok': (c_int, [ctypes.POINTER(ConvGeom), c_int]), 'segnb_conv_upcat_ok': (c_int, [ctypes.POINTER(ConvGeom), c_int, c_int]), 'segnb_conv_fprop_upsum_ok': (c_int, [ctypes.POINTER(ConvGeom), c_int, c_int]), 'segnb_conv_wgrad_bnapply_ok': (c_int, [ctypes.POINTER(ConvGeom), c_int]), 'segnb_upconv_fprop_acc_ok': (c_int, [c_int, c_int, c_int, c_int, c_int, c_int, c_int]), 'segnb_upconv_fprop_ok': (c_int, [c_int, c_int, c_int, c_int, c_int, c_int, c_int]), 'segnb_conv_wgrad_slabs': (c_int, [ctypes.POINTER(ConvGeom), c_int]), 'segnb_pack_job_bytes': (c_int, []), 'segnb_pack_job_blocks': (c_int, [c_int, c_int, c_int, c_ll, c_ll]), 'segnb_device_cus': (c_int, []), 'segnb_last_error': (ctypes.c_char_p, [])}



class McLossSpec(ctypes.Structure):
    _fields_ = [('C', c_int), ('mode', c_int), ('ignore_index', c_ll), ('gamma', c_float), ('w_focal', c_float),
                ('w_nll', c_float), ('w_jaccard', c_float), ('norm', c_float), ('focal_mean', c_int), ('reduce', c_int),
                ('reserved', c_int), ('nll_weight', c_void_p), ('jac_weight', c_void_p)]


MC_SIGNATURES = {
    'segnb_mc_loss_reduce': [_P, _P, c_int, c_int, ctypes.POINTER(McLossSpec), _P, _P, _P],
    'segnb_mc_loss_finalize': [_P, ctypes.POINTER(McLossSpec), _P, _P],
    'segnb_mc_loss_reduce_finalize': [_P, _P, c_int, c_int, ctypes.POINTER(McLossSpec), _P, _P, _P],
    'segnb_mc_loss_bwd': [_P, _P, c_int, c_int, ctypes.POINTER(McLossSpec), _P, _P, _P, _P],
}
MC_PLAIN = {'segnb_mc_loss_work_doubles': (c_int, [c_int])}

GCN_SIGNATURES = {
    'segnb_gcm_fwd': [c_int, _P, c_int, c_int, c_int, c_int, c_int, c_int, _P, _P, _P, _P, _P, _P, _P, _P, _P, _P, _P, _P, _P],
    'segnb_gcm_bwd': [c_int, _P, c_int, c_int, c_int, c_int, c_int, c_int, _P, _P, _P, _P, _P, _P, _P, _P, _P, _P, _P, c_int,
                      _P, _P, _P, _P, _P, _P, _P, _P, _P],
    'segnb_brm_fwd': [c_int, c_int, c_int, c_int, _P, _P, _P, _P, _P, _P, _P, _P],
    'segnb_brm_bwd': [c_int, c_int, c_int, c_int, _P, _P, _P, _P, _P, _P, _P, _P, _P, _P, _P, _P],
    'segnb_resize_bilinear_ac_fwd': [c_int, c_int, c_int, c_int, _P, c_int, c_int, _P, _P, _P],
    'segnb_resize_bilinear_ac_bwd': [c_int, c_int, c_int, c_int, c_int, c_int, _P, _P, _P],
}
GCN_PLAIN = {'segnb_gcn_ok': (c_int, [c_int, c_int, c_int, c_int, c_int])}

_lib = None
_test_backend = None


class NativeLibraryMissing(RuntimeError):
    pass


def load():
    global _lib
    if _lib is not None:
        return _lib
    if not os.path.exists(LIB_PATH):
        raise NativeLibraryMissing(
            'libsegnb_hip.so not found at %s -- build it with __graft_entry__.build() '
            '(segmentation-networks-benchmark_amd/csrc/build.sh); there is no non-HIP path' % LIB_PATH)
    import torch
    lib = ctypes.CDLL(LIB_PATH)
    for name, argtypes in list(SIGNATURES.items()) + list(MC_SIGNATURES.items()) + list(GCN_SIGNATURES.items()):
        fn = getattr(lib, name)
        fn.argtypes = argtypes
        fn.restype = c_int
    for name, (res, argtypes) in list(PLAIN.items()) + list(MC_PLAIN.items()) + list(GCN_PLAIN.items()):
        fn = getattr(lib, name)
        fn.argtypes = argtypes
        fn.restype = res
    _lib = lib
    return lib


def set_backend_for_testing(backend):
    global _test_backend
    if backend is not None and os.environ.get('SEGNB_TEST_HARNESS') != '1':
        raise RuntimeError('set_backend_for_testing is test infrastructure (SEGNB_TEST_HARNESS=1 not set); the product '
                           'path runs on libsegnb_hip.so only')
    _test_backend = backend


def call(name, *args):
    if _test_backend is not None:
        rc = getattr(_test_backend, name)(*args)
        if rc:
            raise RuntimeError('%s failed (emulator) rc=%s' % (name, rc))
        return
    lib = load()
    rc = getattr(lib, name)(*args)
    if rc != 0:
        msg = lib.segnb_last_error()
        raise RuntimeError('HIP error encountered in %s (status %d): %s'
                           % (name, rc, msg.decode() if msg else ''))


def has_test_backend():
    return _test_backend is not None


def plan_record_begin():
    call('segnb_plan_begin')


def plan_record_end():
    h, n = c_void_p(), c_int()
    call('segnb_plan_end', ctypes.byref(h), ctypes.byref(n))
    return (h.value or None), n.value


def plan_record_abort():
    try:
        handle, _ = plan_record_end()
    except Exception:
        return
    if handle is not None:
        try:
            call('segnb_plan_destroy', handle)
        except Exception:
            pass


def census_read():
    if _test_backend is not None:
        return {}
    buf = ctypes.create_string_buffer(1 << 16)
    call('segnb_debug_census', buf, len(buf))
    out = {}
    for line in buf.value.decode().splitlines():
        k, _, v = line.rpartition(' ')
        if not k or not v.isdigit():
            continue
        out[k] = int(v)
    return out


def query(name, *args):
    if _test_backend is not None:
        return getattr(_test_backend, name)(*args)
    return getattr(load(), name)(*args)


def ptr(t, offset_elems=0):
    if t is None:
        return None
    return t.data_ptr() + offset_elems * t.element_size()
# ... 9 lines not shown
```

segmentation-networks-benchmark_amd/segnb/bnpass.py:

```python
import os

import torch

from . import _native as nv

BN_EPS, BN_MOMENTUM = 1e-5, 0.1
STAT_REPLICAS = 16

FUSE_FINALIZE = os.environ.get('SEGNB_FUSE_FINALIZE', '1') != '0'


def _pl(v):
    return (None, 0) if v is None else (v.ptr, v.ld)


def _dp(t):
    return nv.ptr(None if t is None else t.detach())


def module_params(bn, eps=None, momentum=None):
    eps = float(getattr(bn, 'eps', BN_EPS)) if eps is None else eps
    momentum = float(getattr(bn, 'momentum', BN_MOMENTUM) or BN_MOMENTUM) if momentum is None else momentum
    return lambda: (bn.weight, bn.bias, bn.running_mean, bn.running_var, getattr(bn, 'num_batches_tracked', None), eps, momentum)

# ... 8 lines not shown
        self.C, self.Cp, self.act, self.slope, self.params, self.grads, self.accumulate = C, Cp, act, slope, params, grads, accumulate
        self.stats = zeros((STAT_REPLICAS, 2, Cp), torch.float64)
        self.sums = zeros((STAT_REPLICAS, 2, Cp), torch.float64)
        self.coef, self.bcoef = zeros((4, Cp), torch.float32), zeros((3, Cp), torch.float32)
        self.stats_left = self.fused_fwd = False

    def _geom(self, code, y, with_c=True):
        return (code, y.ptr, y.ld, y.N, y.H, y.W) + ((self.C, self.Cp) if with_c else (self.Cp,))

    def _fwd_params(self, *lead):
        gamma, beta, rm, rv, nbt, eps, mom = self.params()
        return lead + (_dp(gamma), _dp(beta), eps, mom, nv.ptr(rm), nv.ptr(rv), nv.ptr(nbt))

    def _bwd_params(self, clear_stats=True):
        dgamma, dbeta = self.grads()
        if clear_stats:
            self.stats_left = False
        return (nv.ptr(self.coef), nv.ptr(self.sums), _dp(self.params()[0]), nv.ptr(self.bcoef), nv.ptr(dgamma), nv.ptr(dbeta),
                self.accumulate, nv.ptr(self.stats) if clear_stats else None)

    def _coef(self):
        return self.coef if self.params is not None else None

    def producer(self, y):
        return (y, self._coef(), self.sums, self.act, self.slope)

    def stats_of(self, code, stream, x):
        nv.call('segnb_bn_stats', code, x.ptr, x.ld, x.N, x.H, x.W, self.Cp, nv.ptr(self.stats), stream)

    def finalize(self, stream, count, train):
        nv.call('segnb_bn_finalize', *(self._fwd_params(nv.ptr(self.stats), self.C, self.Cp, float(count))
                                       + (1 if train else 0, nv.ptr(self.coef), stream)))

    def finalize_keep(self, stream, count):
        nv.call('segnb_bn_finalize_keep', *(self._fwd_params(nv.ptr(self.stats), self.C, self.Cp, float(count))
                                            + (nv.ptr(self.coef), nv.ptr(self.sums), stream)))
        self.stats_left = self.fused_fwd = True

    def act_fwd(self, code, stream, y, out, coef, act, slope, dropmul=None, pool_out=None, up_out=None, res=None):
        nv.call('segnb_bn_act_fwd', *(self._geom(code, y, False) + (nv.ptr(coef), act, slope, nv.ptr(dropmul)) + _pl(out)
                                      + _pl(pool_out) + _pl(up_out) + _pl(res) + (stream,)))

    def forward(self, code, stream, y, fused, train=True, dropmul=None, out=None, pool_out=None, up_out=None, res=None,
                out_stats=None, stats_src=None, head=None):
        self.fused_fwd = bool(fused)
        if fused or head is not None:
            tail = (nv.ptr(self.coef), nv.ptr(self.sums), self.act, self.slope, nv.ptr(dropmul)) + _pl(out)
        if head is not None:
            head_w, head_b, K, logits = head
            nv.call('segnb_bn_fwd_fused_head', *(self._geom(code, y) + self._fwd_params(nv.ptr(self.stats)) + tail
                                                 + (nv.ptr(head_w), nv.ptr(head_b), K, nv.ptr(logits), stream)))
            self.stats_left = True
        elif fused and stats_src is not None:
            nv.call('segnb_bn_fwd_fused_ld', *(self._geom(code, y) + self._fwd_params(nv.ptr(stats_src[0], stats_src[1]), stats_src[2])
                                               + tail + (stream,)))
        elif fused:
            nv.call('segnb_bn_fwd_fused', *(self._geom(code, y) + self._fwd_params(nv.ptr(self.stats)) + tail + _pl(pool_out)
                                            + _pl(up_out) + _pl(res) + (stream,)))
            self.stats_left = True
        else:
            if self.params is not None:
                self.finalize(stream, y.N * y.H * y.W, train)
            if out_stats is not None and pool_out is None and up_out is None and res is None:
                nv.call('segnb_bn_act_fwd_stats', *(self._geom(code, y, False) + (nv.ptr(self._coef()), self.act, self.slope, nv.ptr(dropmul))
                                                    + _pl(out) + (nv.ptr(out_stats[0], out_stats[1]), out_stats[2], stream)))
                return True
            self.act_fwd(code, stream, y, out, self._coef(), self.act, self.slope, dropmul, pool_out, up_out, res)
        return False

    def reduce(self, code, stream, y, g=None, g2=None, g_pool=None, g_up=None, dropmul=None, dz=None, store=True, res=None):
        head = self._geom(code, y, False) + (nv.ptr(self._coef()), self.act, self.slope, nv.ptr(dropmul))
        dzp = (dz.ptr if store else None, dz.ld) if dz is not None else (None, 0)
        if g2 is not None:
            nv.call('segnb_bn_act_bwd_reduce_add', *(head + _pl(g) + _pl(g2) + dzp + (nv.ptr(self.sums),) + _pl(res) + (stream,)))
        else:
            nv.call('segnb_bn_act_bwd_reduce', *(head + _pl(g) + _pl(g_pool) + _pl(g_up) + dzp + (nv.ptr(self.sums),) + _pl(res)
                                                 + (stream,)))

    def head_reduce(self, code, stream, y, dropmul, head_w, K, dlogits, dz, store, dw, db):
        nv.call('segnb_head_bn_bwd', *(self._geom(code, y) + (nv.ptr(self.coef), self.act, self.slope, nv.ptr(dropmul), nv.ptr(head_w),
                                                                K, nv.ptr(dlogits), dz.ptr if store else None, dz.ld, nv.ptr(self.sums),
                                                                nv.ptr(dw), nv.ptr(db), stream)))

    def apply(self, code, stream, y, dy, fused, g=None, dz=None, acc=False, src=None, head=None, clear_stats=True):
        if not fused:
            self.bwd_finalize(stream, y.N * y.H * y.W)
            if g is not None:
                nv.call('segnb_bn_bwd_apply_direct', *(self._geom(code, y, False) + (nv.ptr(self.coef), nv.ptr(self.bcoef), self.act,
                                                                                     self.slope) + _pl(g) + _pl(dy) + (None, self.C, stream)))
            else:
                nv.call('segnb_bn_bwd_apply', *(self._geom(code, y, False) + (nv.ptr(self.coef), nv.ptr(self.bcoef)) + _pl(dz) + _pl(dy)
                                                + (None, self.C, stream)))
            return
        args = self._geom(code, y) + self._bwd_params(clear_stats)
        if head is not None:
            dropmul, head_w, K, dlogits = head
            name, args = 'segnb_head_bn_bwd_apply', args + (self.act, self.slope, nv.ptr(dropmul), nv.ptr(head_w), K, nv.ptr(dlogits))
        elif g is not None:
            name, args = 'segnb_bn_bwd_apply_fused_direct', args + (self.act, self.slope) + _pl(g)
        elif src is not None:
            name = 'segnb_bn_bwd_apply_fused_src'
            args += (self.act, self.slope, nv.ptr(src[0])) + _pl(src[1]) + _pl(src[2]) + _pl(src[3])
        else:
            name, args = 'segnb_bn_bwd_apply_fused', args + _pl(dz)
        nv.call(name + ('_acc' if acc else ''), *(args + _pl(dy) + (stream,)))

    def bwd_finalize(self, stream, count, gbias=None, clear_stats=False):
        if self.params is None:
            nv.call('segnb_bn_bwd_finalize', nv.ptr(self.sums), self.C, self.Cp, float(count), None, nv.ptr(self.coef),
                    nv.ptr(self.bcoef), None, nv.ptr(gbias), 1, stream)
            return
        dgamma, dbeta = self.grads()
        args = (nv.ptr(self.sums), self.C, self.Cp, float(count), _dp(self.params()[0]), nv.ptr(self.coef), nv.ptr(self.bcoef),
                nv.ptr(dgamma), nv.ptr(dbeta), self.accumulate)
        if clear_stats:
            nv.call('segnb_bn_bwd_finalize_clear', *(args + (nv.ptr(self.stats), stream)))
            self.stats_left = False
        else:
            nv.call('segnb_bn_bwd_finalize', *(args + (stream,)))
```

segmentation-networks-benchmark_amd/segnb/engine.py:

```python
import contextlib
import os

import numpy as np
import torch

from . import _native as nv
from . import convplan as cp
from .bnpass import BN_EPS, BN_MOMENTUM, FUSE_FINALIZE, BnLayer, module_params



class KernelTimer(object):

    def __init__(self):
        self.records = []
        self.acc = {}
        self.executed, self.algorithmic = {}, {}
        self.persistent = False

    def launch(self, label, flops, fn, executed=None):
        self.executed[label] = self.executed.get(label, 0.0) + (flops if executed is None else executed)
        self.algorithmic[label] = self.algorithmic.get(label, 0.0) + flops
        a = torch.cuda.Event(enable_timing=True)
        b = torch.cuda.Event(enable_timing=True)
# ... 995 lines not shown
                nv.call('segnb_pack_weight', nv.ptr(j['w']), nv.ptr(j['packed']), j['dtype'], j['Mp'], j['Cp'],
                        j['ntaps'], j['s_m'], j['s_c'], tap, nv.ptr(j['mmap']), nv.ptr(j['cmap']), self.rt.stream)
            else:
                nv.call('segnb_unpack_wgrad', nv.ptr(j['packed']), nv.ptr(j['w']), j['Mp'], j['Cp'], j['ntaps'],
                        j['s_m'], j['s_c'], tap, nv.ptr(j['mmap']), nv.ptr(j['cmap']), 1, self.rt.stream)


class Stage(object):

    direct_apply = True
    recompute_dz_min_mb = 0.0

    fuse_finalize = FUSE_FINALIZE

    def __init__(self, rt, conv, bn=None, act=nv.ACT_RELU, slope=0.01, name=''):
        self.rt, self.conv, self.bn, self.act, self.slope, self.name = rt, conv, bn, act, slope, name
        self.defer_unpack = False
        self.C, self.Cp = conv.Co, conv.Cop
        self.bnl = BnLayer(conv.Co, conv.Cop, rt.zeros, act, slope, module_params(bn, BN_EPS, BN_MOMENTUM) if bn is not None else None)
        self._bufs = {}

    def buffers(self, N, Ho, Wo):
        key = (N, Ho, Wo)
        b = self._bufs.get(key)
        if b is None:
            b = {'y': View.alloc(self.rt, N, Ho, Wo, self.Cp), 'dz': View.alloc(self.rt, N, Ho, Wo, self.Cp)}
            self._bufs[key] = b
        return b

    def defer_act_ok(self, xv, train, need_grad):
        return bool(self.bn is not None and train and need_grad and self.fuse_finalize and self.consumer_fusion)

    consumer_fusion = os.environ.get('SEGNB_CONSUMER_FUSION', '1') != '0'

    def forward(self, xv, train, dropmul=None, out=None, pool_out=None, up_out=None, need_grad=True, u8=None, x_tf=None,
                defer_act=False):
        rt = self.rt
        Ho, Wo = self.conv.out_hw(xv.H, xv.W)
        b = self.buffers(xv.N, Ho, Wo)
        yv = b['y']
        bnl = self.bnl
        use_batch_stats = self.bn is not None and train
        if use_batch_stats and bnl.stats_left:
            bnl.stats.zero_()
            bnl.stats_left = False
        if (not need_grad and not use_batch_stats and u8 is None and out is not None and pool_out is None and up_out is None
                and dropmul is None and self.conv.act_epilogue_ok(xv.H, xv.W)):
            coef = None
            if self.bn is not None:
                bnl.finalize(rt.stream, xv.N * Ho * Wo, False)
                coef = bnl.coef
            self.conv.fprop(xv, out, None, epilogue=(coef, self.act, self.slope))
            self._saved = None
            return out
        self._x_tf = x_tf
        if u8 is not None:
            self.conv.fprop_u8(u8[0], u8[1], yv, bnl.stats if use_batch_stats else None, xv if need_grad else None)
        elif x_tf is not None:
            self.conv.fprop_tf(xv, x_tf, yv, bnl.stats if use_batch_stats else None)
        else:
            self.conv.fprop(xv, yv, bnl.stats if use_batch_stats else None)
        fused = use_batch_stats and self.fuse_finalize and need_grad
        self._saved = (xv, yv, dropmul, self.bn is not None)
        if defer_act == 'head':
            assert fused and pool_out is None and up_out is None
            bnl.stats_left = bnl.fused_fwd = True
        elif defer_act:
            assert fused and dropmul is None and pool_out is None and up_out is None
            bnl.finalize_keep(rt.stream, xv.N * Ho * Wo)
        else:
            bnl.forward(rt.code, rt.stream, yv, fused, train, dropmul, out, pool_out, up_out)
        return yv

    def head_forward(self, head_w, head_b, K, logits, out=None):
        xv, yv, dropmul, _ = self._saved
        self.bnl.forward(self.rt.code, self.rt.stream, yv, True, True, dropmul, out, head=(head_w, head_b, K, logits))

    def head_backward(self, head_w, K, dlogits, dw, db):
        xv, yv, dropmul, _ = self._saved
        dz = self.buffers(yv.N, yv.H, yv.W)['dz']
        self._head_src = (head_w, K, dlogits) if (self.head_dz_recompute and self.bn is not None and self.fuse_finalize) else None
        self.bnl.head_reduce(self.rt.code, self.rt.stream, yv, dropmul, head_w, K, dlogits, dz, self._head_src is None, dw, db)

    head_dz_recompute = os.environ.get('SEGNB_HEAD_DZ', '1') != '0'
    _head_src = None

    def tf_out(self):
        return ConvOp.tf_act(self.bnl.coef, self.Cp, self.act, self.slope)

    def reduce_in_producer(self):
        xv, yv, dropmul, has_bn = self._saved
        if not (self.direct_apply and has_bn and dropmul is None and self.bnl.fused_fwd):
            return None
        return self.bnl.producer(yv)

    def backward(self, grads, g_direct=None, g_pool=None, g_up=None, dx=None, reduced=False, fuse_reduce_of=None,
                 dz_ready=False):
        rt, bnl = self.rt, self.bnl
        xv, yv, dropmul, has_bn = self._saved
        dz = self.buffers(yv.N, yv.H, yv.W)['dz']
        fused = has_bn and bnl.fused_fwd
        if has_bn:
            bnl.grads = lambda: (grads.grad_of(self.bn.weight), grads.grad_of(self.bn.bias))
        direct = (self.direct_apply and has_bn and g_direct is not None and g_pool is None and g_up is None
                  and dropmul is None and not dz_ready)
        assert not reduced or direct, 'only a direct layer can be reduced by its producer'
        mb = yv.N * yv.H * yv.W * self.Cp * (2 if rt.code == nv.BF16 else 4) / 1e6
        recompute = (not direct and not dz_ready and fused and self.recompute_dz_min_mb > 0 and mb >= self.recompute_dz_min_mb)
        if not reduced and not dz_ready:
            bnl.reduce(rt.code, rt.stream, yv, g_direct, None, g_pool, g_up, dropmul, dz, store=not (direct or recompute))
        count = yv.N * yv.H * yv.W
        if (dx is None and direct and fused and self.defer_unpack
                and isinstance(self.conv, ConvOp) and self.conv.wgrad_bnapply_ok(xv, yv)):
            bnl.bwd_finalize(rt.stream, count, clear_stats=True)
            self.conv.wgrad_bnapply(xv, g_direct, yv, bnl.coef, bnl.bcoef, self.act, self.slope,
                                    grad_w=grads.grad_of(self.conv.weight))
            return False
        if self.defer_unpack and dx is not None and rt.side_stream() is not None:
            rt.arm_fork()
        if not has_bn:
            bnl.bwd_finalize(rt.stream, count, gbias=grads.grad_of(self.conv.bias) if self.conv.bias is not None else None)
        elif dz_ready and self._head_src is not None and fused:
            bnl.apply(rt.code, rt.stream, yv, dz, True, head=(dropmul,) + self._head_src)
        elif direct:
            bnl.apply(rt.code, rt.stream, yv, dz, fused, g=g_direct)
        elif recompute:
            bnl.apply(rt.code, rt.stream, yv, dz, True, src=(dropmul, g_direct, g_pool, g_up))
        else:
            bnl.apply(rt.code, rt.stream, yv, dz, fused, dz=dz)
        x_tf = getattr(self, '_x_tf', None)

        def wgrad(unpack):
            if x_tf is not None:
                assert self.defer_unpack and not unpack
                self.conv.wgrad_tf(xv, x_tf, dz, None, grad_w=grads.grad_of(self.conv.weight))
            else:
                self.conv.wgrad(xv, dz, grads.grad_of(self.conv.weight), unpack=unpack)
        side = rt.fork_side() if (self.defer_unpack and dx is not None) else None
        if side is not None:
            with torch.cuda.stream(side):
                wgrad(False)
        else:
            wgrad(not self.defer_unpack)
        fused = False
        if dx is not None:
            ep = fuse_reduce_of.reduce_in_producer() if fuse_reduce_of is not None else None
            if ep is not None and self.conv.dgrad_bnreduce_ok(dz, dx):
                self.conv.dgrad(dz, dx, bn_reduce=ep)
                fused = True
            else:
                self.conv.dgrad(dz, dx)
        return fused


class FlatParams(object):

    registry = {}

    def __init__(self, module):
        self.module = module
        self.flat_p = None
        self.flat_g = None
        self._off = {}
        self._gviews = {}
        self._slots = None
        self.version = 0

    def _structure(self):
        if self._slots is None:
            ps, bs, seen = [], [], set()
            for m in self.module.modules():
                for n, p in m._parameters.items():
                    if p is not None and id(p) not in seen:
                        seen.add(id(p))
                        ps.append((m, n))
                for n, b in m._buffers.items():
                    if b is not None and id(b) not in seen:
                        seen.add(id(b))
                        bs.append((m, n))
            self._slots = (ps, bs)
        return self._slots

    def forget_structure(self):
        self._slots = None
        self._modules = None

    _modules = None

    def module_list(self):
        if self._modules is None:
            self._modules = list(self.module.modules())
        return self._modules

    def param_list(self):
        out = [m._parameters[n] for m, n in self._structure()[0]]
        if any(p is None for p in out):
            self._slots = None
            out = [m._parameters[n] for m, n in self._structure()[0]]
        return out

    def buffer_list(self):
        out = [m._buffers[n] for m, n in self._structure()[1]]
        if any(b is None for b in out):
# ... 121 lines not shown
```

segmentation-networks-benchmark_amd/segnb/seglosses.py:

```python
import weakref

import os

import torch

from . import _native as nv

SPEC_FIELDS = ('w_bce', 'w_focal', 'w_jaccard', 'w_sjaccard', 'w_dice', 'smooth', 'eps', 'norm', 'focal_mean',
               'bce_sum', 'focal_gamma')


def make_spec(w_bce=0.0, w_focal=0.0, w_jaccard=0.0, w_sjaccard=0.0, w_dice=0.0, smooth=100.0, eps=1e-7,
              norm=1.0, focal_mean=0, bce_sum=0, focal_gamma=2.0):
    return (float(w_bce), float(w_focal), float(w_jaccard), float(w_sjaccard), float(w_dice), float(smooth),
            float(eps), float(norm), int(focal_mean), int(bce_sum), float(focal_gamma))


def _cspec(spec):
    s = nv.LossSpec()
    for k, v in zip(SPEC_FIELDS, spec):
        setattr(s, k, v)
    return s


def _stream(t):
    return torch.cuda.current_stream(t.device).cuda_stream if t.is_cuda else 0


class DataParallelHooks(object):
    sums_allreduce = None
    grad_scale = 1.0

    @classmethod
    def reset(cls):
        cls.sums_allreduce, cls.grad_scale = None, 1.0


def _prep(logits, target):
    if logits.shape != target.shape:
        raise ValueError('logits %s and target %s must have the same shape'
                         % (tuple(logits.shape), tuple(target.shape)))
    x = logits.detach().contiguous().float()
    t = target.detach()
    if t.dtype != torch.int64:
        t = t.to(torch.int64)
    return x, t.contiguous()


_last = None


def _remember(logits, target, fin):
    global _last
    try:
        _last = (weakref.ref(logits), logits._version, weakref.ref(target), target._version, fin)
    except TypeError:
        _last = None


def _recall(logits, target):
    if _last is None:
        return None
    rl, vl, rt, vt, fin = _last
    if rl() is logits and rt() is target and logits._version == vl and target._version == vt:
        return fin
    return None


_grad_buffers = {}


def register_grad_buffer(logits, buf):
    _grad_buffers.clear()
    _grad_buffers[logits.data_ptr()] = buf


def _grad_buffer_for(x):
    buf = _grad_buffers.pop(x.data_ptr(), None)
    if buf is not None and buf.shape == x.shape and buf.dtype == x.dtype and buf.device == x.device:
        return buf
    return None


_ONE_LAUNCH = True
_loss_work = {}


def reduce_finalize(x, t, spec):
    fin = torch.empty(8, dtype=torch.float32, device=x.device)
    st = _stream(x)
    if DataParallelHooks.sums_allreduce is None and _ONE_LAUNCH:
        key = (x.device.index, st)
        work = _loss_work.get(key)
        if work is None:
            work = _loss_work[key] = torch.zeros(128, dtype=torch.float64, device=x.device)
        try:
            nv.call('segnb_seg_loss_reduce_finalize', nv.ptr(x), nv.ptr(t), x.numel(), _cspec(spec), nv.ptr(work), nv.ptr(fin), st)
        except BaseException:
            _loss_work.pop(key, None)
            raise
        return work, fin
    sums = torch.zeros(8, dtype=torch.float64, device=x.device)
    nv.call('segnb_seg_loss_reduce', nv.ptr(x), nv.ptr(t), x.numel(), float(spec[10]), nv.ptr(sums), st)
    if DataParallelHooks.sums_allreduce is not None:
        DataParallelHooks.sums_allreduce(sums)
    cs = _cspec(spec)
    nv.call('segnb_seg_loss_finalize', nv.ptr(sums), cs, nv.ptr(fin), st)
    return sums, fin


class SegLossFn(torch.autograd.Function):
    @staticmethod
    def forward(ctx, logits, target, spec):
        x, t = _prep(logits, target)
        sums, fin = reduce_finalize(x, t, spec)
        ctx.spec = spec
        ctx.save_for_backward(x, t, sums, fin)
        SegLossFn.last_fin = fin
        return fin[0]

    @staticmethod
    def backward(ctx, gout):
        x, t, sums, fin = ctx.saved_tensors
        g = gout.detach().contiguous().float()
        if DataParallelHooks.grad_scale != 1.0:
            g = g * DataParallelHooks.grad_scale
        dx = _grad_buffer_for(x)
        if dx is None:
            dx = torch.empty_like(x)
        cs = _cspec(ctx.spec)
        nv.call('segnb_seg_loss_bwd', nv.ptr(x), nv.ptr(t), x.numel(), nv.ptr(sums), nv.ptr(fin), cs, nv.ptr(g),
                nv.ptr(dx), _stream(x))
        return dx, None, None


def seg_loss(logits, target, spec):
    out = SegLossFn.apply(logits, target, spec)
    _remember(logits, target, SegLossFn.last_fin)
    SegLossFn.last_fin = None
    return out


def seg_metrics(logits, target):
    fin = _recall(logits, target)
    if fin is None:
        x, t = _prep(logits, target)
        _, fin = reduce_finalize(x, t, make_spec(w_bce=1.0))
        _remember(logits, target, fin)
    return fin[1].clone(), fin[2].clone()


class SegLossMapFn(torch.autograd.Function):

    @staticmethod
    def forward(ctx, logits, target, kind, gamma):
        x, t = _prep(logits, target)
        out = torch.empty_like(x)
        nv.call('segnb_seg_loss_map', nv.ptr(x), nv.ptr(t), x.numel(), kind, float(gamma), nv.ptr(out), _stream(x))
        ctx.cfg = (kind, float(gamma))
        ctx.save_for_backward(x, t)
        return out

    @staticmethod
    def backward(ctx, gout):
        x, t = ctx.saved_tensors
        kind, gamma = ctx.cfg
        g = gout.detach().contiguous().float()
        dx = torch.empty_like(x)
        nv.call('segnb_seg_loss_map_bwd', nv.ptr(x), nv.ptr(t), x.numel(), kind, gamma, nv.ptr(g), nv.ptr(dx), _stream(x))
        return dx, None, None, None


def seg_loss_map(logits, target, kind, gamma=2.0):
    return SegLossMapFn.apply(logits, target, kind, gamma)
```

Baseline: 6903 images/s.

## Fuse segmentation loss gradient into head BN backward kernel

The loss backward can now skip its separate gradient kernel and pass a deferred loss source to the head layer. The head BN backward kernel then computes each pixel's loss gradient inline from logits and targets, so the dlogits tensor is never written and read back. It also adds a ticket-based last-block fold that sums the per-block dw/db partials inside the same kernel, replacing a separate finish launch. In exchange the code is more complex: an atomic ticket counter lives in a scratch header, and the fusion relies on single-class heads and a fragile token handshake between autograd and the engine.

```diff
diff --git a/__graft_entry__.py b/__graft_entry__.py
--- a/__graft_entry__.py
+++ b/__graft_entry__.py
@@ -20,7 +20,7 @@
     import ctypes
     lib = ctypes.CDLL(nv.LIB_PATH)
     for name in (list(nv.SIGNATURES) + list(nv.PLAIN) + list(nv.MC_SIGNATURES) + list(nv.MC_PLAIN) + list(nv.GCN_SIGNATURES)
-                 + list(nv.GCN_PLAIN)):
+                 + list(nv.GCN_PLAIN) + list(nv.HL_SIGNATURES)):
         getattr(lib, name)
     import lib.models.zf_unet
     import lib.models.gcn
diff --git a/include/segnb_head_loss.h b/include/segnb_head_loss.h
--- /dev/null
+++ b/include/segnb_head_loss.h
@@ -0,0 +1,30 @@
+#ifndef SEGNB_HEAD_LOSS_H
+#define SEGNB_HEAD_LOSS_H
+
+#include "segnb_hip.h"
+
+#ifdef __cplusplus
+extern "C" {
+#endif
+
+typedef struct {
+    const float* logits;
+    const long long* target;
+    const float* fin;
+    const float* grad_out;
+    segnb_loss_spec spec;
+} segnb_head_loss_src;
+
+int segnb_head_bn_bwd_loss(int dtype, const void* y, int ld_y, int N, int H, int W, int C, int Cp, const float* coef, int act,
+                           float slope, const float* dropmul, const float* head_w, const segnb_head_loss_src* src,
+                           float* dlogits_out, double* sums, float* dw, float* db, segnb_stream_t stream);
+int segnb_head_bn_bwd_apply_loss(int dtype, const void* y, int ld_y, int N, int H, int W, int C, int Cp, const float* coef,
+                                 const double* sums, const float* gamma, float* bcoef, float* dgamma, float* dbeta,
+                                 int accumulate, double* fwd_stats_to_clear, int act, float slope, const float* dropmul,
+                                 const float* head_w, const segnb_head_loss_src* src, void* dy, int ld_dy,
+                                 segnb_stream_t stream);
+
+#ifdef __cplusplus
+}
+#endif
+#endif
diff --git a/segmentation-networks-benchmark_amd/csrc/common.h b/segmentation-networks-benchmark_amd/csrc/common.h
--- a/segmentation-networks-benchmark_amd/csrc/common.h
+++ b/segmentation-networks-benchmark_amd/csrc/common.h
@@ -132,6 +132,7 @@
 int segnb_knob_fprop_rw();
 int segnb_knob_fprop_ksplit();
 float* segnb_head_scratch(size_t bytes, hipStream_t stream);
+unsigned* segnb_head_ticket(float* scratch);
 void segnb_head_bwd_finish(const float* part, int gx, int gy, int K, int C, int CT, float* dw, float* db, hipStream_t stream);
 int segnb_knob_pack_blocks();
 int segnb_knob_fprop_roll();
diff --git a/segmentation-networks-benchmark_amd/csrc/head_loss.hip b/segmentation-networks-benchmark_amd/csrc/head_loss.hip
--- a/segmentation-networks-benchmark_amd/csrc/head_loss.hip
+++ b/segmentation-networks-benchmark_amd/csrc/head_loss.hip
@@ -1,4 +1,5 @@
 #include "common.h"
+#include "loss_grad.h"
 
 #include <mutex>
 #include <vector>
@@ -489,37 +490,6 @@
             db[k / T] += tot;
         }
     }
-}
-
-struct PixTerms {
-    float p;
-    float e;
-    float de;
-    float f;
-    float df;
-};
-
-__device__ __forceinline__ PixTerms pix_terms(float x, float t, float gamma = 2.f) {
-    PixTerms o;
-    const float ls = fminf(x, 0.f) - log1pf(expf(-fabsf(x)));
-    const float p = expf(ls);
-    o.p = p;
-    o.e = -t * ls + log1pf(p);
-    o.de = (1.f - p) * (p / (1.f + p) - t);
-    const float pt = expf(-o.e);
-    const float om = 1.f - pt;
-    if (gamma == 2.f) {
-        o.f = om * om * o.e;
-        o.df = (2.f * om * pt * o.e + om * om) * o.de;
-    } else if (om > 0.f) {
-        const float pg1 = powf(om, gamma - 1.f), pg = pg1 * om;
-        o.f = pg * o.e;
-        o.df = (gamma * pg1 * pt * o.e + pg) * o.de;
-    } else {
-        o.f = gamma == 0.f ? o.e : 0.f;
-        o.df = gamma == 0.f ? o.de : 0.f;
-    }
-    return o;
 }
 
 __device__ __forceinline__ void loss_finalize_math(const double* sums, const segnb_loss_spec& sp, float* __restrict__ out) {
@@ -640,17 +610,8 @@
                                                        long long n, const float* __restrict__ fin, segnb_loss_spec sp,
                                                        const float* __restrict__ grad_out, float* __restrict__ dx,
                                                        int vec) {
-    const float go = (grad_out != nullptr ? grad_out[0] : 1.f) / sp.norm;
-    const float GI = fin[3], GU = fin[4];
-    const float inv_n = 1.f / fin[6];
-    const float wb = sp.bce_sum ? sp.w_bce : sp.w_bce * inv_n;
-    const float wf = sp.focal_mean ? sp.w_focal * inv_n : sp.w_focal;
-    auto grad = [&](float xv, long long tgv) {
-        const float tf = (float)tgv;
-        const PixTerms q = pix_terms(xv, tf, sp.focal_gamma);
-        const float dp = q.p * (1.f - q.p);
-        return go * (wb * q.de + wf * q.df + dp * (tf * GI + GU));
-    };
+    const LossGradScalars lg = loss_grad_scalars(fin, sp, grad_out);
+    auto grad = [&](float xv, long long tgv) { return loss_grad_pixel(lg, xv, tgv); };
     const long long n4 = vec ? n / 4 : 0;
     for (long long j = blockIdx.x * (long long)blockDim.x + threadIdx.x; j < n4; j += (long long)gridDim.x * blockDim.x) {
         const float4 xv = reinterpret_cast<const float4*>(x)[j];
@@ -785,6 +746,7 @@
 }
 
 namespace {
+constexpr int HEAD_SCRATCH_HDR = 64;
 float* head_scratch(size_t bytes, hipStream_t stream) {
     struct Ent {
         int dev;
@@ -818,11 +780,12 @@
     if (bytes > e->cap) {
         const size_t want = bytes < (1u << 20) ? (1u << 20) : bytes * 2;
         float* p = nullptr;
-        if (hipMalloc(&p, want) != hipSuccess) {
+        if (hipMalloc(&p, want + HEAD_SCRATCH_HDR * sizeof(float)) != hipSuccess ||
+            hipMemsetAsync(p, 0, HEAD_SCRATCH_HDR * sizeof(float), stream) != hipSuccess) {
             segnb_set_error("segnb_head_bwd: scratch allocation of %zu bytes failed", want);
             return nullptr;
         }
-        e->buf = p;
+        e->buf = p + HEAD_SCRATCH_HDR;
         e->cap = want;
     }
     return e->buf;
@@ -830,6 +793,7 @@
 }
 
 float* segnb_head_scratch(size_t bytes, hipStream_t stream) { return head_scratch(bytes, stream); }
+unsigned* segnb_head_ticket(float* scratch) { return reinterpret_cast<unsigned*>(scratch - HEAD_SCRATCH_HDR); }
 void segnb_head_bwd_finish(const float* part, int gx, int gy, int K, int C, int CT, float* dw, float* db, hipStream_t stream) {
     head_bwd_finish_kernel<<<dim3(K * C + K), dim3(256), 0, stream>>>(part, gx, gy, K, C, CT, dw, db, 1);
 }
diff --git a/segmentation-networks-benchmark_amd/csrc/loss_grad.h b/segmentation-networks-benchmark_amd/csrc/loss_grad.h
--- /dev/null
+++ b/segmentation-networks-benchmark_amd/csrc/loss_grad.h
@@ -0,0 +1,65 @@
+#pragma once
+#include "common.h"
+
+struct PixTerms {
+    float p;
+    float e;
+    float de;
+    float f;
+    float df;
+};
+
+static __device__ __forceinline__ PixTerms pix_terms(float x, float t, float gamma = 2.f) {
+    PixTerms o;
+    const float ls = fminf(x, 0.f) - log1pf(expf(-fabsf(x)));
+    const float p = expf(ls);
+    o.p = p;
+    o.e = -t * ls + log1pf(p);
+    o.de = (1.f - p) * (p / (1.f + p) - t);
+    const float pt = expf(-o.e);
+    const float om = 1.f - pt;
+    if (gamma == 2.f) {
+        o.f = om * om * o.e;
+        o.df = (2.f * om * pt * o.e + om * om) * o.de;
+    } else if (om > 0.f) {
+        const float pg1 = powf(om, gamma - 1.f), pg = pg1 * om;
+        o.f = pg * o.e;
+        o.df = (gamma * pg1 * pt * o.e + pg) * o.de;
+    } else {
+        o.f = gamma == 0.f ? o.e : 0.f;
+        o.df = gamma == 0.f ? o.de : 0.f;
+    }
+    return o;
+}
+
+struct LossGradScalars {
+    float go, GI, GU, wb, wf, gamma;
+};
+
+static __device__ __forceinline__ LossGradScalars loss_grad_scalars(const float* __restrict__ fin, const segnb_loss_spec& sp,
+                                                                    const float* __restrict__ grad_out) {
+    LossGradScalars c;
+    c.go = (grad_out != nullptr ? grad_out[0] : 1.f) / sp.norm;
+    c.GI = fin[3];
+    c.GU = fin[4];
+    const float inv_n = 1.f / fin[6];
+    c.wb = sp.bce_sum ? sp.w_bce : sp.w_bce * inv_n;
+    c.wf = sp.focal_mean ? sp.w_focal * inv_n : sp.w_focal;
+    c.gamma = sp.focal_gamma;
+    return c;
+}
+
+static __device__ __forceinline__ float loss_grad_pixel(const LossGradScalars& c, float xv, long long tgv) {
+    const float tf = (float)tgv;
+    const PixTerms q = pix_terms(xv, tf, c.gamma);
+    const float dp = q.p * (1.f - q.p);
+    return c.go * (c.wb * q.de + c.wf * q.df + dp * (tf * c.GI + c.GU));
+}
+
+struct HeadLossSrc {
+    const float* x;
+    const long long* tg;
+    const float* fin;
+    const float* grad_out;
+    segnb_loss_spec sp;
+};
diff --git a/segmentation-networks-benchmark_amd/csrc/norm_act.hip b/segmentation-networks-benchmark_amd/csrc/norm_act.hip
--- a/segmentation-networks-benchmark_amd/csrc/norm_act.hip
+++ b/segmentation-networks-benchmark_amd/csrc/norm_act.hip
@@ -1,4 +1,6 @@
 #include "common.h"
+#include "loss_grad.h"
+#include "../../include/segnb_head_loss.h"
 
 namespace {
 
@@ -803,136 +805,128 @@
     }
 }
 
-template <typename T, int KM>
+template <int U>
+struct LossTrip {
+    float x[U];
+    long long t[U];
+};
+template <int U>
+__device__ __forceinline__ void loss_trip_issue(LossTrip<U>& lt, const HeadLossSrc& ls, int it0, int stride, int npix, int tx,
+                                                int CT) {
+#pragma unroll
+    for (int r = 0; r < U; ++r) {
+        if (r * CT < U) {
+            const int uo = r * CT + tx;
+            const int pix = it0 + (uo < U ? uo : 0) * stride;
+            const int pc = pix < npix ? pix : it0;
+            lt.x[r] = ls.x[pc];
+            lt.t[r] = ls.tg[pc];
+        }
+    }
+}
+template <int U>
+__device__ __forceinline__ void loss_trip_grads(const LossTrip<U>& lt, const LossGradScalars& lg, int it0, int stride, int npix,
+                                                int tx, int CT, float* __restrict__ out, float (&g)[U]) {
+    float gv[U];
+#pragma unroll
+    for (int r = 0; r < U; ++r) {
+        gv[r] = 0.f;
+        if (r * CT < U) {
+            gv[r] = loss_grad_pixel(lg, lt.x[r], lt.t[r]);
+            const int uo = r * CT + tx;
+            const int pix = it0 + uo * stride;
+            if (out != nullptr && uo < U && pix < npix) out[pix] = gv[r];
+        }
+    }
+    const int base = (int)(threadIdx.x & 63) - tx;
+#pragma unroll
+    for (int u = 0; u < U; ++u) {
+        const int r = u / CT;
+        float v = gv[0];
+#pragma unroll
+        for (int rr = 1; rr < U; ++rr) v = r == rr ? gv[rr] : v;
+        g[u] = __shfl(v, base + (u - r * CT), 64);
+    }
+}
+
+constexpr int FOLD_G = 17;
+constexpr int FOLD_T = 8;
+__device__ __forceinline__ void head_fold_finish(const float* __restrict__ part, int gx, int K, int C, int CT, unsigned* ticket,
+                                                 float* __restrict__ dw, float* __restrict__ db, float* sred) {
+    __shared__ int last;
+    asm volatile("s_waitcnt vmcnt(0)" ::: "memory");
+    __syncthreads();
+    if (threadIdx.x == 0) {
+        const unsigned tk = __hip_atomic_fetch_add(ticket, 1u, __ATOMIC_RELAXED, __HIP_MEMORY_SCOPE_AGENT);
+        last = tk == gridDim.x * gridDim.y - 1 ? 1 : 0;
+        if (last) {
+            __hip_atomic_store(ticket, 0u, __ATOMIC_RELAXED, __HIP_MEMORY_SCOPE_AGENT);
+            __builtin_amdgcn_fence(__ATOMIC_ACQUIRE, "agent");
+            asm volatile("s_waitcnt vmcnt(0)" ::: "memory");
+        }
+    }
+    __syncthreads();
+    if (!last) return;
+    const int t = threadIdx.x, lane = t & 63, wave = t >> 6;
+    const int row = K * (CT * 8 + 1), nout = K * C + K;
+    for (int o0 = 0; o0 < nout; o0 += FOLD_G) {
+        float v[FOLD_T][FOLD_G];
+        int col[FOLD_G];
+#pragma unroll
+        for (int q = 0; q < FOLD_G; ++q) {
+            const int o = o0 + q < nout ? o0 + q : nout - 1;
+            if (o < K * C) {
+                const int k = o / C, c = o - k * C, by = c / (CT * 8);
+                col[q] = by * gx * row + k * (CT * 8 + 1) + (c - by * (CT * 8));
+            } else {
+                col[q] = (o - K * C) * (CT * 8 + 1) + CT * 8;
+            }
+        }
+#pragma unroll
+        for (int j = 0; j < FOLD_T; ++j) {
+            const int bx = t + j * NTHR;
+#pragma unroll
+            for (int q = 0; q < FOLD_G; ++q)
+                v[j][q] = bx < gx ? __hip_atomic_load(part + (long long)bx * row + col[q], __ATOMIC_RELAXED, __HIP_MEMORY_SCOPE_AGENT)
+                                  : 0.f;
+        }
+        __syncthreads();
+#pragma unroll
+        for (int q = 0; q < FOLD_G; ++q) {
+            float sum = 0.f;
+#pragma unroll
+            for (int j = 0; j < FOLD_T; ++j)
+                if (t + j * NTHR < gx) sum += v[j][q];
+#pragma unroll
+            for (int d = 32; d >= 1; d >>= 1) sum += __shfl_down(sum, d, 64);
+            if (lane == 0) sred[wave * FOLD_G + q] = sum;
+        }
+        __syncthreads();
+        if (t < FOLD_G && o0 + t < nout) {
+            const int o = o0 + t;
+            const float tot = ((sred[t] + sred[FOLD_G + t]) + sred[2 * FOLD_G + t]) + sred[3 * FOLD_G + t];
+            if (o < K * C) {
+                if (dw != nullptr) dw[o] += tot;
+            } else if (db != nullptr) {
+                db[o - K * C] += tot;
+            }
+        }
+    }
+}
+
+template <typename T, int KM, bool LS = false>
 __global__ __launch_bounds__(NTHR) void head_bn_bwd_kernel(const T* __restrict__ y, int ld_y, EwShape s,
                                                            const float* __restrict__ coef, int act, float slope,
                                                            const float* __restrict__ dropmul, const float* __restrict__ w, int C,
                                                            int K, const float* __restrict__ dl, T* __restrict__ dz, int ld_dz,
-                                                           double* __restrict__ sums, float* __restrict__ part) {
+                                                           double* __restrict__ sums, float* __restrict__ part,
+                                                           const HeadLossSrc ls, float* __restrict__ dl_out,
+                                                           unsigned* __restrict__ ticket, float* __restrict__ dw,
+                                                           float* __restrict__ db) {
+    static_assert(!LS || KM == 1, "the loss-source form serves one class");
     __shared__ float sred[SRED_FLOATS];
-    constexpr int U = 2;
-    const int tx = threadIdx.x % s.CT, ty = threadIdx.x / s.CT;
-    const int cc = blockIdx.y * s.CT + tx;
-    const bool active = cc < s.CPP;
-    const int c0 = active ? cc * 8 : 0;
-    const int stride = gridDim.x * s.PY;
-    const int npix = s.N * s.H * s.W, hw = s.H * s.W;
-    const FastDiv d_hw(hw);
-    float wv[KM][8], gw[KM][8], gb[KM];
-#pragma unroll
-    for (int k = 0; k < KM; ++k) {
-        gb[k] = 0.f;
-#pragma unroll
-        for (int e = 0; e < 8; ++e) {
-            wv[k][e] = (k < K && c0 + e < C) ? w[k * C + c0 + e] : 0.f;
-            gw[k][e] = 0.f;
-        }
-    }
-    float sc[8], sh[8], mu[8], s1[8], s2[8];
-    load8(coef + c0, sc);
-    load8(coef + s.Cp + c0, sh);
-    load8(coef + 2 * s.Cp + c0, mu);
-#pragma unroll
-    for (int e = 0; e < 8; ++e) s1[e] = s2[e] = 0.f;
-    if (active) {
-        for (int it0 = blockIdx.x * s.PY + ty; it0 < npix; it0 += U * stride) {
-            Raw8<T> ry[U];
-            Raw8<float> rdm[U];
-            float g[U][KM];
-#pragma unroll
-            for (int u = 0; u < U; ++u) {
-                const int pix = it0 + u * stride;
-                const int pc = pix < npix ? pix : it0;
-                load_raw(y + (long long)pc * ld_y + c0, ry[u]);
-                const int n = (dropmul != nullptr || KM > 1) ? d_hw.div(pc) : 0;
-                if (dropmul != nullptr) load_raw(dropmul + n * s.Cp + c0, rdm[u]);
-                if (KM == 1) {
-                    g[u][0] = dl[pc];
-                } else {
-                    const int r = pc - n * hw;
-#pragma unroll
-                    for (int k = 0; k < KM; ++k) g[u][k] = k < K ? dl[((long long)n * K + k) * hw + r] : 0.f;
-                }
-            }
-#pragma unroll
-            for (int u = 0; u < U; ++u) {
-                const int pix = it0 + u * stride;
-                if (pix >= npix) break;
-                float yv[8], dm[8], a[8], d[8], yc[8], z[8];
-                unpack_raw(ry[u], yv);
-#pragma unroll
-                for (int e = 0; e < 8; ++e) dm[e] = 1.f;
-                if (dropmul != nullptr) unpack_raw(rdm[u], dm);
-#pragma unroll
-                for (int e = 0; e < 8; ++e) {
-                    yc[e] = yv[e] - mu[e];
-                    z[e] = yc[e] * sc[e] + sh[e];
-                    a[e] = dm[e] * act_fwd(z[e], act, slope);
-                    d[e] = 0.f;
-                }
-                round_store8((T*)nullptr, a);
-#pragma unroll
-                for (int k = 0; k < KM; ++k)
-                    if (k < K) {
-                        const float gk = g[u][k];
-                        gb[k] += gk;
-#pragma unroll
-                        for (int e = 0; e < 8; ++e) {
-                            d[e] = fmaf(gk, wv[k][e], d[e]);
-                            gw[k][e] = fmaf(gk, a[e], gw[k][e]);
-                        }
-                    }
-                round_store8((T*)nullptr, d);
-#pragma unroll
-                for (int e = 0; e < 8; ++e) d[e] = d[e] * dm[e] * act_grad(z[e] + 0.f, act, slope);
-                round_store8(dz != nullptr ? dz + (long long)pix * ld_dz + c0 : (T*)nullptr, d);
-#pragma unroll
-                for (int e = 0; e < 8; ++e) {
-                    s1[e] += d[e];
-                    s2[e] += d[e] * yc[e];
-                }
-            }
-        }
-    }
-#pragma unroll
-    for (int e = 0; e < 8; ++e) s2[e] *= coef[3 * s.Cp + c0 + e];
-    double* rep = sums + (long long)(blockIdx.x % REPL) * 2 * s.Cp;
-    block_channel_sum2(s1, s2, s, tx, blockIdx.y * s.CT, rep, rep + s.Cp, sred);
-    const int CT = s.CT, PY = s.PY;
-    float* sg = sred;
-    float* prow = part + (long long)(blockIdx.y * gridDim.x + blockIdx.x) * (K * (CT * 8 + 1));
-#pragma unroll
-    for (int k = 0; k < KM; ++k)
-        if (k < K) {
-            __syncthreads();
-#pragma unroll
-            for (int e = 0; e < 8; ++e) sg[(ty * CT + tx) * 8 + e] = gw[k][e];
-            __syncthreads();
-            if ((int)threadIdx.x < CT * 8) {
-                float sum = 0.f;
-                for (int j = 0; j < PY; ++j) sum += sg[j * CT * 8 + threadIdx.x];
-                prow[k * (CT * 8 + 1) + threadIdx.x] = sum;
-            }
-            __syncthreads();
-            if (tx == 0) sg[ty] = gb[k];
-            __syncthreads();
-            if (threadIdx.x == 0) {
-                float sum = 0.f;
-                for (int j = 0; j < PY; ++j) sum += sg[j];
-                prow[k * (CT * 8 + 1) + CT * 8] = sum;
-            }
-        }
-}
-
-
-template <typename T, int KM>
-__global__ __launch_bounds__(NTHR) void head_bn_apply_kernel(const T* __restrict__ y, int ld_y, EwShape s,
-                                                             const float* __restrict__ coef, int act, float slope,
-                                                             const float* __restrict__ dropmul, const float* __restrict__ w, int C,
-                                                             int K, const float* __restrict__ dl, T* __restrict__ dy, int ld_dy,
-                                                             const BnBwdParams bp) {
-    __shared__ float sred[SRED_FLOATS];
-    constexpr int U = 2;
+    __shared__ float sgb[NTHR];
+    constexpr int U = LS ? 4 : 2;
     const int tx = threadIdx.x % s.CT, ty = threadIdx.x / s.CT;
     const int cc = blockIdx.y * s.CT + tx;
     const bool active = cc < s.CPP;
@@ -943,6 +937,7 @@
     Raw8<T> ry[U];
     Raw8<float> rdm[U];
     float g[U][KM];
+    LossTrip<U> lt;
     auto issue = [&](int it0) {
 #pragma unroll
         for (int u = 0; u < U; ++u) {
@@ -951,7 +946,8 @@
             load_raw(y + (long long)pc * ld_y + c0, ry[u]);
             const int n = (dropmul != nullptr || KM > 1) ? d_hw.div(pc) : 0;
             if (dropmul != nullptr) load_raw(dropmul + n * s.Cp + c0, rdm[u]);
-            if (KM == 1) {
+            if constexpr (LS) {
+            } else if (KM == 1) {
                 g[u][0] = dl[pc];
             } else {
                 const int r = pc - n * hw;
@@ -959,9 +955,152 @@
                 for (int k = 0; k < KM; ++k) g[u][k] = k < K ? dl[((long long)n * K + k) * hw + r] : 0.f;
             }
         }
+        if constexpr (LS) loss_trip_issue(lt, ls, it0, stride, npix, tx, s.CT);
     };
     int it0 = blockIdx.x * s.PY + ty;
     if (active && it0 < npix) issue(it0);
+    LossGradScalars lg = {};
+    if constexpr (LS) lg = loss_grad_scalars(ls.fin, ls.sp, ls.grad_out);
+    float wv[KM][8], gw[KM][8], gb[KM];
+#pragma unroll
+    for (int k = 0; k < KM; ++k) {
+        gb[k] = 0.f;
+#pragma unroll
+        for (int e = 0; e < 8; ++e) {
+            wv[k][e] = (k < K && c0 + e < C) ? w[k * C + c0 + e] : 0.f;
+            gw[k][e] = 0.f;
+        }
+    }
+    float sc[8], sh[8], mu[8], s1[8], s2[8];
+    load8(coef + c0, sc);
+    load8(coef + s.Cp + c0, sh);
+    load8(coef + 2 * s.Cp + c0, mu);
+#pragma unroll
+    for (int e = 0; e < 8; ++e) s1[e] = s2[e] = 0.f;
+    if (active) {
+        while (it0 < npix) {
+            if constexpr (LS) {
+                float gl[U];
+                loss_trip_grads(lt, lg, it0, stride, npix, tx, s.CT, blockIdx.y == 0 ? dl_out : (float*)nullptr, gl);
+#pragma unroll
+                for (int u = 0; u < U; ++u) g[u][0] = gl[u];
+            }
+#pragma unroll
+            for (int u = 0; u < U; ++u) {
+                const int pix = it0 + u * stride;
+                if (pix >= npix) break;
+                float yv[8], dm[8], a[8], d[8], yc[8], z[8];
+                unpack_raw(ry[u], yv);
+#pragma unroll
+                for (int e = 0; e < 8; ++e) dm[e] = 1.f;
+                if (dropmul != nullptr) unpack_raw(rdm[u], dm);
+#pragma unroll
+                for (int e = 0; e < 8; ++e) {
+                    yc[e] = yv[e] - mu[e];
+                    z[e] = yc[e] * sc[e] + sh[e];
+                    a[e] = dm[e] * act_fwd(z[e], act, slope);
+                    d[e] = 0.f;
+                }
+                round_store8((T*)nullptr, a);
+#pragma unroll
+                for (int k = 0; k < KM; ++k)
+                    if (k < K) {
+                        const float gk = g[u][k];
+                        gb[k] += gk;
+#pragma unroll
+                        for (int e = 0; e < 8; ++e) {
+                            d[e] = fmaf(gk, wv[k][e], d[e]);
+                            gw[k][e] = fmaf(gk, a[e], gw[k][e]);
+                        }
+                    }
+                round_store8((T*)nullptr, d);
+#pragma unroll
+                for (int e = 0; e < 8; ++e) d[e] = d[e] * dm[e] * act_grad(z[e] + 0.f, act, slope);
+                round_store8(dz != nullptr ? dz + (long long)pix * ld_dz + c0 : (T*)nullptr, d);
+#pragma unroll
+                for (int e = 0; e < 8; ++e) {
+                    s1[e] += d[e];
+                    s2[e] += d[e] * yc[e];
+                }
+            }
+            it0 += U * stride;
+            if (it0 < npix) issue(it0);
+        }
+    }
+#pragma unroll
+    for (int e = 0; e < 8; ++e) s2[e] *= coef[3 * s.Cp + c0 + e];
+    double* rep = sums + (long long)(blockIdx.x % REPL) * 2 * s.Cp;
+    block_channel_sum2(s1, s2, s, tx, blockIdx.y * s.CT, rep, rep + s.Cp, sred);
+    const int CT = s.CT, PY = s.PY;
+    float* sg = sred;
+    float* prow = part + (long long)(blockIdx.y * gridDim.x + blockIdx.x) * (K * (CT * 8 + 1));
+#pragma unroll
+    for (int k = 0; k < KM; ++k)
+        if (k < K) {
+            __syncthreads();
+#pragma unroll
+            for (int e = 0; e < 8; ++e) sg[(ty * CT + tx) * 8 + e] = gw[k][e];
+            if (tx == 0) sgb[ty] = gb[k];
+            __syncthreads();
+            for (int i = threadIdx.x; i <= CT * 8; i += NTHR) {
+                const bool isw = i < CT * 8;
+                const float* src = isw ? sg + i : sgb;
+                const int step = isw ? CT * 8 : 1;
+                float sum = 0.f;
+#pragma unroll 8
+                for (int j = 0; j < PY; ++j) sum += src[j * step];
+                float* dst = prow + k * (CT * 8 + 1) + i;
+                if constexpr (LS) __hip_atomic_store(dst, sum, __ATOMIC_RELAXED, __HIP_MEMORY_SCOPE_AGENT);
+                else *dst = sum;
+            }
+        }
+    if constexpr (LS) head_fold_finish(part, (int)gridDim.x, K, C, CT, ticket, dw, db, sred);
+}
+
+
+template <typename T, int KM, bool LS = false>
+__global__ __launch_bounds__(NTHR) void head_bn_apply_kernel(const T* __restrict__ y, int ld_y, EwShape s,
+                                                             const float* __restrict__ coef, int act, float slope,
+                                                             const float* __restrict__ dropmul, const float* __restrict__ w, int C,
+                                                             int K, const float* __restrict__ dl, T* __restrict__ dy, int ld_dy,
+                                                             const BnBwdParams bp, const HeadLossSrc ls) {
+    static_assert(!LS || KM == 1, "the loss-source form serves one class");
+    __shared__ float sred[SRED_FLOATS];
+    constexpr int U = LS ? 4 : 2;
+    const int tx = threadIdx.x % s.CT, ty = threadIdx.x / s.CT;
+    const int cc = blockIdx.y * s.CT + tx;
+    const bool active = cc < s.CPP;
+    const int c0 = active ? cc * 8 : 0;
+    const int stride = gridDim.x * s.PY;
+    const int npix = s.N * s.H * s.W, hw = s.H * s.W;
+    const FastDiv d_hw(hw);
+    Raw8<T> ry[U];
+    Raw8<float> rdm[U];
+    float g[U][KM];
+    LossTrip<U> lt;
+    auto issue = [&](int it0) {
+#pragma unroll
+        for (int u = 0; u < U; ++u) {
+            const int pix = it0 + u * stride;
+            const int pc = pix < npix ? pix : it0;
+            load_raw(y + (long long)pc * ld_y + c0, ry[u]);
+            const int n = (dropmul != nullptr || KM > 1) ? d_hw.div(pc) : 0;
+            if (dropmul != nullptr) load_raw(dropmul + n * s.Cp + c0, rdm[u]);
+            if constexpr (LS) {
+            } else if (KM == 1) {
+                g[u][0] = dl[pc];
+            } else {
+                const int r = pc - n * hw;
+#pragma unroll
+                for (int k = 0; k < KM; ++k) g[u][k] = k < K ? dl[((long long)n * K + k) * hw + r] : 0.f;
+            }
+        }
+        if constexpr (LS) loss_trip_issue(lt, ls, it0, stride, npix, tx, s.CT);
+    };
+    int it0 = blockIdx.x * s.PY + ty;
+    if (active && it0 < npix) issue(it0);
+    LossGradScalars lg = {};
+    if constexpr (LS) lg = loss_grad_scalars(ls.fin, ls.sp, ls.grad_out);
     float ap[4][8];
     apply_src_coefs(bp, coef, s, tx, c0, sred, ap);
     float wv[KM][8];
@@ -975,6 +1114,12 @@
     load8(coef + 2 * s.Cp + c0, mu);
     if (!active) return;
     while (it0 < npix) {
+        if constexpr (LS) {
+            float gl[U];
+            loss_trip_grads(lt, lg, it0, stride, npix, tx, s.CT, (float*)nullptr, gl);
+#pragma unroll
+            for (int u = 0; u < U; ++u) g[u][0] = gl[u];
+        }
 #pragma unroll
         for (int u = 0; u < U; ++u) {
             const int pix = it0 + u * stride;
@@ -1659,7 +1804,8 @@
     if (part == nullptr) return SEGNB_E_BADARG;
 #define SEGNB_HBB(TT, KMM)                                                                                          \
     hipLaunchKernelGGL((head_bn_bwd_kernel<TT, KMM>), grid, dim3(NTHR), 0, (hipStream_t)stream, (const TT*)y, ld_y, s, coef, \
-                       act, slope, dropmul, head_w, C, K, dlogits, (TT*)dz, ld_dz, sums, part)
+                       act, slope, dropmul, head_w, C, K, dlogits, (TT*)dz, ld_dz, sums, part, HeadLossSrc{}, (float*)nullptr,        \
+                       (unsigned*)nullptr, (float*)nullptr, (float*)nullptr)
     if (dtype == SEGNB_BF16) {
         if (K == 1) SEGNB_HBB(bf16_t, 1); else SEGNB_HBB(bf16_t, 4);
     } else if (dtype == SEGNB_F32) {
@@ -1693,7 +1839,7 @@
     const BnBwdParams bp = {sums, (double)N * H * W, gamma, dgamma, dbeta, C, accumulate, bcoef, fwd_stats_to_clear};
 #define SEGNB_HBA(TT, KMM)                                                                                                    \
     SEGNB_LAUNCH_FORKABLE((head_bn_apply_kernel<TT, KMM>), grid, dim3(NTHR), 0, (hipStream_t)stream, (const TT*)y, ld_y, s, coef, \
-                          act, slope, dropmul, head_w, C, K, dlogits, (TT*)dy, ld_dy, bp)
+                          act, slope, dropmul, head_w, C, K, dlogits, (TT*)dy, ld_dy, bp, HeadLossSrc{})
     if (dtype == SEGNB_BF16) {
         if (K == 1) SEGNB_HBA(bf16_t, 1); else SEGNB_HBA(bf16_t, 4);
     } else if (dtype == SEGNB_F32) {
@@ -1703,6 +1849,82 @@
         return SEGNB_E_BADARG;
     }
 #undef SEGNB_HBA
+    SEGNB_LAUNCH_CHECK();
+    return 0;
+}
+
+static int head_loss_src_check(const segnb_head_loss_src* src, const EwShape& s, const char* fn) {
+    if (src == nullptr || src->logits == nullptr || src->target == nullptr || src->fin == nullptr || src->spec.norm == 0.f) {
+        segnb_set_error("%s: bad argument: incomplete loss source", fn);
+        return SEGNB_E_BADARG;
+    }
+    if (s.CPP != s.CT) {
+        segnb_set_error("%s: bad argument: Cp / 8 must be a power of two <= 32", fn);
+        return SEGNB_E_BADARG;
+    }
+    return 0;
+}
+
+extern "C" int segnb_head_bn_bwd_loss(int dtype, const void* y, int ld_y, int N, int H, int W, int C, int Cp, const float* coef,
+                                      int act, float slope, const float* dropmul, const float* head_w,
+                                      const segnb_head_loss_src* src, float* dlogits_out, double* sums, float* dw, float* db,
+                                      segnb_stream_t stream) {
+    SEGNB_PLAN_REFUSE("segnb_head_bn_bwd_loss reads tensors whose addresses change from step to step");
+    if (int rc = check_ew(N, H, W, Cp)) return rc;
+    SEGNB_CHECK_ARG(y && coef && head_w && sums && dlogits_out && C > 0 && Cp >= C, "NULL tensor");
+    SEGNB_CHECK_ARG(segnb_head_fused_ok(1, Cp), "Cp / 8 a power of two <= 32 (segnb_head_fused_ok)");
+    SEGNB_CHECK_ARG(ld_y % 8 == 0 && ld_y >= Cp, "bad strides");
+    const EwShape s = make_shape(N, H, W, Cp);
+    if (int rc = head_loss_src_check(src, s, "segnb_head_bn_bwd_loss")) return rc;
+    const dim3 grid = make_grid(s, (long long)N * H * W);
+    SEGNB_CHECK_ARG(grid.y == 1 && grid.x <= (unsigned)(NTHR * FOLD_T), "grid outside the folded finish");
+    float* part = segnb_head_scratch((size_t)grid.x * grid.y * (s.CT * 8 + 1) * sizeof(float), (hipStream_t)stream);
+    if (part == nullptr) return SEGNB_E_BADARG;
+    const HeadLossSrc ls = {src->logits, src->target, src->fin, src->grad_out, src->spec};
+#define SEGNB_HBL(TT)                                                                                                          \
+    hipLaunchKernelGGL((head_bn_bwd_kernel<TT, 1, true>), grid, dim3(NTHR), 0, (hipStream_t)stream, (const TT*)y, ld_y, s, coef, \
+                       act, slope, dropmul, head_w, C, 1, (const float*)nullptr, (TT*)nullptr, 0, sums, part, ls, dlogits_out,   \
+                       segnb_head_ticket(part), dw, db)
+    if (dtype == SEGNB_BF16) {
+        SEGNB_HBL(bf16_t);
+    } else if (dtype == SEGNB_F32) {
+        SEGNB_HBL(float);
+    } else {
+        segnb_set_error("segnb_head_bn_bwd_loss: unknown dtype %d", dtype);
+        return SEGNB_E_BADARG;
+    }
+#undef SEGNB_HBL
+    SEGNB_LAUNCH_CHECK();
+    return 0;
+}
+
+extern "C" int segnb_head_bn_bwd_apply_loss(int dtype, const void* y, int ld_y, int N, int H, int W, int C, int Cp,
+                                            const float* coef, const double* sums, const float* gamma, float* bcoef,
+                                            float* dgamma, float* dbeta, int accumulate, double* fwd_stats_to_clear, int act,
+                                            float slope, const float* dropmul, const float* head_w,
+                                            const segnb_head_loss_src* src, void* dy, int ld_dy, segnb_stream_t stream) {
+    SEGNB_PLAN_REFUSE("segnb_head_bn_bwd_apply_loss reads tensors whose addresses change from step to step");
+    if (int rc = check_ew(N, H, W, Cp)) return rc;
+    SEGNB_CHECK_ARG(y && coef && sums && bcoef && head_w && dy && C > 0 && Cp >= C, "NULL tensor");
+    SEGNB_CHECK_ARG(segnb_head_fused_ok(1, Cp), "Cp / 8 a power of two <= 32 (segnb_head_fused_ok)");
+    SEGNB_CHECK_ARG(ld_y % 8 == 0 && ld_dy % 8 == 0 && ld_y >= Cp && ld_dy >= Cp, "bad strides");
+    const EwShape s = make_shape(N, H, W, Cp);
+    if (int rc = head_loss_src_check(src, s, "segnb_head_bn_bwd_apply_loss")) return rc;
+    const dim3 grid = make_grid(s, (long long)N * H * W);
+    const BnBwdParams bp = {sums, (double)N * H * W, gamma, dgamma, dbeta, C, accumulate, bcoef, fwd_stats_to_clear};
+    const HeadLossSrc ls = {src->logits, src->target, src->fin, src->grad_out, src->spec};
+#define SEGNB_HAL(TT)                                                                                                              \
+    SEGNB_LAUNCH_FORKABLE((head_bn_apply_kernel<TT, 1, true>), grid, dim3(NTHR), 0, (hipStream_t)stream, (const TT*)y, ld_y, s, coef, \
+                          act, slope, dropmul, head_w, C, 1, (const float*)nullptr, (TT*)dy, ld_dy, bp, ls)
+    if (dtype == SEGNB_BF16) {
+        SEGNB_HAL(bf16_t);
+    } else if (dtype == SEGNB_F32) {
+        SEGNB_HAL(float);
+    } else {
+        segnb_set_error("segnb_head_bn_bwd_apply_loss: unknown dtype %d", dtype);
+        return SEGNB_E_BADARG;
+    }
+#undef SEGNB_HAL
     SEGNB_LAUNCH_CHECK();
     return 0;
 }
diff --git a/segmentation-networks-benchmark_amd/lib/models/zf_unet.py b/segmentation-networks-benchmark_amd/lib/models/zf_unet.py
--- a/segmentation-networks-benchmark_amd/lib/models/zf_unet.py
+++ b/segmentation-networks-benchmark_amd/lib/models/zf_unet.py
@@ -499,8 +499,13 @@
         else:
             nv.call('segnb_head_fwd', rt.code, b['f0'].ptr, b['f0'].ld, N, H, W, self.widths[0],
                     nv.ptr(head.weight.detach()), nv.ptr(head.bias.detach()), self.K, nv.ptr(logits), rt.stream)
-        seglosses.register_grad_buffer(logits, b['dlogits_in'])
+        s2 = self.stages[DECODER[-1]][1]
+        self_eval = self.generation if (fused and self.K == 1 and self.HEAD_LOSS_FUSION and s2.head_loss_ok()
+                                        and rt.device.type == 'cuda' and not nv.has_test_backend()) else None
+        seglosses.register_grad_buffer(logits, b['dlogits_in'], self_eval=self_eval)
         return logits
+
+    HEAD_LOSS_FUSION = os.environ.get('SEGNB_HEAD_LOSS_FUSION', '1') != '0'
 
     def backward(self, dlogits):
         self._guard_mode, self._guard_active = (None, None), False
@@ -525,19 +530,30 @@
         rt, flat, wp = self.rt, self.flat, self.wp
         drop_now = {n: self.stages[n][1]._saved[2] if self.stages[n][1]._saved is not None else None for n in ENCODER + DECODER}
         ckey = self._cplan_key('bwd', N, H, W, True, True, drop_now)
+        from segnb import seglosses
+        hf = bool(getattr(self, '_last_head_fused', False))
+        din = b['dlogits_in']
+        src = seglosses.take_source(self.generation, din)
+        if src is not None and not (hf and dlogits.data_ptr() == din.data_ptr()):
+            raise RuntimeError('the loss left d(loss)/d(logits) to the model, but the gradient that arrived is not the registered '
+                               'buffer (something besides the loss consumes the logits): run with SEGNB_HEAD_LOSS_FUSION=0')
         if ckey is not None:
-            ckey = ckey + (bool(getattr(self, '_last_head_fused', False)), bool(accumulate_in_place))
+            ckey = ckey + (hf, bool(accumulate_in_place), src is not None)
         if ckey is not None:
-            din = b['dlogits_in']
             if dlogits.data_ptr() != din.data_ptr():
                 din.copy_(dlogits)
             dlogits = din
             plan = self._cplans.get(ckey)
             self._guard_active = self._guard_b.begin()
+        if src is not None:
+            head = self.module.conv_final
+            self.stages[DECODER[-1]][1].head_backward_loss(flat, head.weight.detach(), src.native(), din,
+                                                           flat.grad_of(head.weight), flat.grad_of(head.bias))
+        if ckey is not None:
             if plan is not None and plan[0] is not None:
                 self._guard_mode = (ckey, 'replay')
                 self._plan_replay(plan, H, W)
-                rt._side_busy = False
+                rt._side_busy = rt._armed = False
                 self._after_backward()
                 flat.publish_grads(accumulate_in_place)
                 return [None] * len(flat._off)
@@ -547,8 +563,9 @@
             if self._dg_pack_on_side and rt.side_stream() is not None:
                 nv.call('segnb_stream_join', rt.stream, rt.side_stream().cuda_stream)
             head = self.module.conv_final
-            hf = bool(getattr(self, '_last_head_fused', False))
-            if hf:
+            if src is not None:
+                pass
+            elif hf:
                 self.stages[DECODER[-1]][1].head_backward(head.weight.detach(), self.K, dlogits, flat.grad_of(head.weight),
                                                           flat.grad_of(head.bias))
             else:
@@ -558,7 +575,7 @@
             for name, lvl in zip(reversed(DECODER), (0, 1, 2, 3, 4)):
                 s1, s2 = self.stages[name]
                 if lvl == 0 and hf:
-                    red = s2.backward(flat, dx=b['db1_0'], fuse_reduce_of=s1, dz_ready=True)
+                    red = s2.backward(flat, dx=b['db1_0'], fuse_reduce_of=s1, dz_ready=True, applied=src is not None)
                 elif lvl == 0:
                     red = s2.backward(flat, g_direct=b['df0'], dx=b['db1_0'], fuse_reduce_of=s1)
                 elif self._seg(lvl - 1, N, H, W):
diff --git a/segmentation-networks-benchmark_amd/segnb/_native.py b/segmentation-networks-benchmark_amd/segnb/_native.py
--- a/segmentation-networks-benchmark_amd/segnb/_native.py
+++ b/segmentation-networks-benchmark_amd/segnb/_native.py
@@ -207,6 +207,19 @@
 }
 GCN_PLAIN = {'segnb_gcn_ok': (c_int, [c_int, c_int, c_int, c_int, c_int])}
 
+
+
+class HeadLossSrc(ctypes.Structure):
+    _fields_ = [('logits', c_void_p), ('target', c_void_p), ('fin', c_void_p), ('grad_out', c_void_p), ('spec', LossSpec)]
+
+
+HL_SIGNATURES = {
+    'segnb_head_bn_bwd_loss': [c_int, _P, c_int, c_int, c_int, c_int, c_int, c_int, _P, c_int, c_float, _P, _P,
+                               ctypes.POINTER(HeadLossSrc), _P, _P, _P, _P, _P],
+    'segnb_head_bn_bwd_apply_loss': [c_int, _P, c_int, c_int, c_int, c_int, c_int, c_int, _P, _P, _P, _P, _P, _P, c_int, _P, c_int,
+                                     c_float, _P, _P, ctypes.POINTER(HeadLossSrc), _P, c_int, _P],
+}
+
 _lib = None
 _test_backend = None
 
@@ -225,7 +238,7 @@
             '(segmentation-networks-benchmark_amd/csrc/build.sh); there is no non-HIP path' % LIB_PATH)
     import torch
     lib = ctypes.CDLL(LIB_PATH)
-    for name, argtypes in list(SIGNATURES.items()) + list(MC_SIGNATURES.items()) + list(GCN_SIGNATURES.items()):
+    for name, argtypes in list(SIGNATURES.items()) + list(MC_SIGNATURES.items()) + list(GCN_SIGNATURES.items()) + list(HL_SIGNATURES.items()):
         fn = getattr(lib, name)
         fn.argtypes = argtypes
         fn.restype = c_int
diff --git a/segmentation-networks-benchmark_amd/segnb/bnpass.py b/segmentation-networks-benchmark_amd/segnb/bnpass.py
--- a/segmentation-networks-benchmark_amd/segnb/bnpass.py
+++ b/segmentation-networks-benchmark_amd/segnb/bnpass.py
@@ -114,6 +114,11 @@
                                                                 K, nv.ptr(dlogits), dz.ptr if store else None, dz.ld, nv.ptr(self.sums),
                                                                 nv.ptr(dw), nv.ptr(db), stream)))
 
+    def head_reduce_loss(self, code, stream, y, dropmul, head_w, src, dlogits_out, dw, db):
+        nv.call('segnb_head_bn_bwd_loss', *(self._geom(code, y) + (nv.ptr(self.coef), self.act, self.slope, nv.ptr(dropmul),
+                                                                     nv.ptr(head_w), src, nv.ptr(dlogits_out), nv.ptr(self.sums),
+                                                                     nv.ptr(dw), nv.ptr(db), stream)))
+
     def apply(self, code, stream, y, dy, fused, g=None, dz=None, acc=False, src=None, head=None, clear_stats=True):
         if not fused:
             self.bwd_finalize(stream, y.N * y.H * y.W)
@@ -125,7 +130,10 @@
                                                 + (None, self.C, stream)))
             return
         args = self._geom(code, y) + self._bwd_params(clear_stats)
-        if head is not None:
+        if head is not None and len(head) == 3:
+            dropmul, head_w, src = head
+            name, args = 'segnb_head_bn_bwd_apply_loss', args + (self.act, self.slope, nv.ptr(dropmul), nv.ptr(head_w), src)
+        elif head is not None:
             dropmul, head_w, K, dlogits = head
             name, args = 'segnb_head_bn_bwd_apply', args + (self.act, self.slope, nv.ptr(dropmul), nv.ptr(head_w), K, nv.ptr(dlogits))
         elif g is not None:
diff --git a/segmentation-networks-benchmark_amd/segnb/engine.py b/segmentation-networks-benchmark_amd/segnb/engine.py
--- a/segmentation-networks-benchmark_amd/segnb/engine.py
+++ b/segmentation-networks-benchmark_amd/segnb/engine.py
@@ -1101,6 +1101,20 @@
         self._head_src = (head_w, K, dlogits) if (self.head_dz_recompute and self.bn is not None and self.fuse_finalize) else None
         self.bnl.head_reduce(self.rt.code, self.rt.stream, yv, dropmul, head_w, K, dlogits, dz, self._head_src is None, dw, db)
 
+    def head_backward_loss(self, grads, head_w, src, dlogits_out, dw, db):
+        rt, bnl = self.rt, self.bnl
+        xv, yv, dropmul, _ = self._saved
+        dz = self.buffers(yv.N, yv.H, yv.W)['dz']
+        self._head_src = None
+        bnl.grads = lambda: (grads.grad_of(self.bn.weight), grads.grad_of(self.bn.bias))
+        bnl.head_reduce_loss(rt.code, rt.stream, yv, dropmul, head_w, src, dlogits_out, dw, db)
+        if self.defer_unpack and rt.side_stream() is not None:
+            rt.arm_fork()
+        bnl.apply(rt.code, rt.stream, yv, dz, True, head=(dropmul, head_w, src))
+
+    def head_loss_ok(self):
+        return bool(self.head_dz_recompute and self.bn is not None and self.fuse_finalize and self.bnl.fused_fwd)
+
     head_dz_recompute = os.environ.get('SEGNB_HEAD_DZ', '1') != '0'
     _head_src = None
 
@@ -1114,7 +1128,7 @@
         return self.bnl.producer(yv)
 
     def backward(self, grads, g_direct=None, g_pool=None, g_up=None, dx=None, reduced=False, fuse_reduce_of=None,
-                 dz_ready=False):
+                 dz_ready=False, applied=False):
         rt, bnl = self.rt, self.bnl
         xv, yv, dropmul, has_bn = self._saved
         dz = self.buffers(yv.N, yv.H, yv.W)['dz']
@@ -1135,9 +1149,13 @@
             self.conv.wgrad_bnapply(xv, g_direct, yv, bnl.coef, bnl.bcoef, self.act, self.slope,
                                     grad_w=grads.grad_of(self.conv.weight))
             return False
-        if self.defer_unpack and dx is not None and rt.side_stream() is not None:
+        if applied:
+            assert dz_ready and fused and dx is not None
+        elif self.defer_unpack and dx is not None and rt.side_stream() is not None:
             rt.arm_fork()
-        if not has_bn:
+        if applied:
+            pass
+        elif not has_bn:
             bnl.bwd_finalize(rt.stream, count, gbias=grads.grad_of(self.conv.bias) if self.conv.bias is not None else None)
         elif dz_ready and self._head_src is not None and fused:
             bnl.apply(rt.code, rt.stream, yv, dz, True, head=(dropmul,) + self._head_src)
diff --git a/segmentation-networks-benchmark_amd/segnb/seglosses.py b/segmentation-networks-benchmark_amd/segnb/seglosses.py
--- a/segmentation-networks-benchmark_amd/segnb/seglosses.py
+++ b/segmentation-networks-benchmark_amd/segnb/seglosses.py
@@ -69,17 +69,48 @@
 
 _grad_buffers = {}
 
-
-def register_grad_buffer(logits, buf):
+HEAD_LOSS_FUSION = os.environ.get('SEGNB_HEAD_LOSS_FUSION', '1') != '0'
+
+
+class LossSource(object):
+    __slots__ = ('token', 'logits', 'target', 'fin', 'spec', 'gout', 'buf')
+
+    def native(self):
+        src = nv.HeadLossSrc()
+        src.logits, src.target, src.fin, src.grad_out = nv.ptr(self.logits), nv.ptr(self.target), nv.ptr(self.fin), nv.ptr(self.gout)
+        src.spec = _cspec(self.spec)
+        return src
+
+
+pending_source = None
+
+
+def take_source(token, buf):
+    global pending_source
+    src, pending_source = pending_source, None
+    if src is not None and src.token == token and src.buf is buf:
+        return src
+    return None
+
+
+def register_grad_buffer(logits, buf, self_eval=None):
     _grad_buffers.clear()
-    _grad_buffers[logits.data_ptr()] = buf
-
-
-def _grad_buffer_for(x):
-    buf = _grad_buffers.pop(x.data_ptr(), None)
-    if buf is not None and buf.shape == x.shape and buf.dtype == x.dtype and buf.device == x.device:
-        return buf
-    return None
+    _grad_buffers[logits.data_ptr()] = [buf, self_eval, 0]
+
+
+def _note_use(x):
+    ent = _grad_buffers.get(x.data_ptr())
+    if ent is not None:
+        ent[2] += 1
+
+
+def _grad_buffer_for(x, with_token=False):
+    ent = _grad_buffers.pop(x.data_ptr(), None)
+    if ent is not None:
+        buf, token, uses = ent
+        if buf.shape == x.shape and buf.dtype == x.dtype and buf.device == x.device:
+            return (buf, token if uses == 1 else None) if with_token else buf
+    return (None, None) if with_token else None
 
 
 _ONE_LAUNCH = True
@@ -115,6 +146,11 @@
         x, t = _prep(logits, target)
         sums, fin = reduce_finalize(x, t, spec)
         ctx.spec = spec
+        _note_use(x)
+        try:
+            ctx.logits_ref = weakref.ref(logits)
+        except TypeError:
+            ctx.logits_ref = None
         ctx.save_for_backward(x, t, sums, fin)
         SegLossFn.last_fin = fin
         return fin[0]
@@ -125,13 +161,24 @@
         g = gout.detach().contiguous().float()
         if DataParallelHooks.grad_scale != 1.0:
             g = g * DataParallelHooks.grad_scale
-        dx = _grad_buffer_for(x)
+        dx, token = _grad_buffer_for(x, with_token=True)
         if dx is None:
             dx = torch.empty_like(x)
+        elif token is not None and HEAD_LOSS_FUSION and _self_eval_ok(ctx, x):
+            global pending_source
+            src = pending_source = LossSource()
+            src.token, src.logits, src.target, src.fin, src.spec, src.gout, src.buf = token, x, t, fin, ctx.spec, g, dx
+            return dx, None, None
         cs = _cspec(ctx.spec)
         nv.call('segnb_seg_loss_bwd', nv.ptr(x), nv.ptr(t), x.numel(), nv.ptr(sums), nv.ptr(fin), cs, nv.ptr(g),
                 nv.ptr(dx), _stream(x))
         return dx, None, None
+
+
+def _self_eval_ok(ctx, x):
+    lg = ctx.logits_ref() if ctx.logits_ref is not None else None
+    return bool(lg is not None and x.dim() == 4 and x.shape[1] == 1 and not getattr(lg, '_backward_hooks', None)
+                and not getattr(lg, 'retains_grad', False))
 
 
 def seg_loss(logits, target, spec):
```

Measured after the change: 6783 images/s. 0.983x the previous value.
